# terraytherapeutics/COATI

Measured on AMD Instinct MI355X. Metric: molecules/sec (contrastive+AR train step), grande_closed, higher is better.
Workload: dtype bf16; 1 GPU; grande_closed d=256 L=16 nh=16 + E3GNN h=256x5, V=10322, batch 1024/GPU, seq_len 80, 16-atom point clouds, InfoNCE + AR loss, bf16 MFMA operands / fp32 accumulate + fp32 master weights, random-init weights; global_batch=1024, seq_len=80, parallelism=dp1

## Files before the change

coati_amd/build.py:

```python
import os
import subprocess
import sys
from concurrent.futures import ThreadPoolExecutor

HERE = os.path.dirname(os.path.abspath(__file__))
CSRC = os.path.join(HERE, "csrc")
LIBDIR = os.path.join(HERE, "lib")
LIB = os.path.join(LIBDIR, "libcoati_hip_x.so" if os.environ.get("COATI_AMD_EXPERIMENTAL") == "1" else "libcoati_hip.so")
OBJDIR = os.path.join(HERE, "build")
HIP_UNITS = ["gemm.hip", "gemm_rb.hip", "gemm_rb16.hip", "gemm_ring.hip", "gemm_mx8.hip", "norm.hip", "attention.hip", "attention16.hip", "embed.hip", "gnn.hip", "loss.hip", "optim.hip", "batch.hip", "decode.hip"]
CPP_UNITS = ["engine.cpp", "capi.cpp", "tokenizer.cpp", "comm.cpp"]
FLAGS = ["--offload-arch=gfx950", "-O3", "-std=c++17", "-fPIC", "-Wno-unused-value", "-mllvm", "-amdgpu-mfma-vgpr-form=1"] + os.environ.get("COATI_AMD_CXXFLAGS", "").split()


EXPERIMENTAL = os.environ.get("COATI_AMD_EXPERIMENTAL") == "1"
EXPERIMENTAL_UNITS = ["experimental/attn_block.hip", "experimental/mlp64.hip", "experimental/gemm_t32.hip"]
if EXPERIMENTAL:
    HIP_UNITS = HIP_UNITS + EXPERIMENTAL_UNITS
    FLAGS = FLAGS + ["-DCOATI_EXPERIMENTAL"]
UNIT_DROP_FLAGS = {"experimental/mlp64.hip": ("-mllvm", "-amdgpu-mfma-vgpr-form=1")}


def _hipcc():
    for c in (os.environ.get("HIPCC"), "/opt/rocm/bin/hipcc", "hipcc"):
        if c and (os.path.isabs(c) and os.path.exists(c) or not os.path.isabs(c)):
            return c
    return "hipcc"


def _sources():
    deps = [os.path.join(CSRC, f) for f in os.listdir(CSRC) if not os.path.isdir(os.path.join(CSRC, f))]
    if EXPERIMENTAL:
        deps += [os.path.join(CSRC, "experimental", f) for f in os.listdir(os.path.join(CSRC, "experimental"))]
    deps.append(os.path.join(os.path.dirname(HERE), "include", "coati_hip.h"))
    return deps


def _stamp_path():
    return LIB + ".flags"


def needs_build():
    if not os.path.exists(LIB):
        return True
    try:
        with open(_stamp_path()) as f:
            if f.read() != " ".join(FLAGS):
                return True
    except OSError:
        return True
    t = os.path.getmtime(LIB)
    return any(os.path.getmtime(p) > t for p in _sources())


def build(force=False, verbose=True):
    if not force and not needs_build():
        return LIB
    os.makedirs(LIBDIR, exist_ok=True)
    os.makedirs(OBJDIR, exist_ok=True)
    import fcntl
    with open(os.path.join(LIBDIR, ".build.lock"), "w") as lock:
        fcntl.flock(lock, fcntl.LOCK_EX)
        try:
            if not force and not needs_build():
                return LIB
            return _build_locked(verbose)
        finally:
            fcntl.flock(lock, fcntl.LOCK_UN)


def _build_locked(verbose):
    hipcc = _hipcc()

    def compile_one(unit):
        src = os.path.join(CSRC, unit)
        obj = os.path.join(OBJDIR, unit.replace("/", "_") + (".x.o" if EXPERIMENTAL else ".o"))
        flags = [f for f in FLAGS if f not in UNIT_DROP_FLAGS.get(unit, ())]
        cmd = [hipcc] + flags + (["-x", "hip"] if unit.endswith(".cpp") else []) + ["-c", src, "-o", obj]
        r = subprocess.run(cmd, capture_output=True, text=True)
        if r.returncode != 0:
            raise RuntimeError(f"hipcc failed on {unit}:\n{r.stderr}")
        return obj

    with ThreadPoolExecutor(max_workers=8) as ex:
        objs = list(ex.map(compile_one, HIP_UNITS + CPP_UNITS))
    tmp = LIB + f".tmp{os.getpid()}"
    r = subprocess.run([hipcc, "--offload-arch=gfx950", "-shared", "-fPIC"] + objs + ["-lpthread", "-ldl", "-o", tmp], capture_output=True, text=True)
    if r.returncode != 0:
        raise RuntimeError(f"link failed:\n{r.stderr}")
    os.replace(tmp, LIB)
    with open(_stamp_path(), "w") as f:
        f.write(" ".join(FLAGS))
    if verbose:
        print(f"[coati_amd] built {LIB}", file=sys.stderr)
    return LIB


if __name__ == "__main__":
    build(force="--force" in sys.argv)
```

coati_amd/csrc/engine.cpp:

```cpp
#include <stdarg.h>
#include <stdio.h>
#include <stdlib.h>
#include <string.h>

#include <algorithm>
#include <string>
#include <vector>

#include "../../include/coati_hip.h"
#include "kernels.h"

#define HIPCHK(x) do { hipError_t _h = (x); if (_h != hipSuccess) { coati_set_error("%s: %s", #x, hipGetErrorString(_h)); return COATI_EHIP; } } while (0)

static thread_local char g_err[512] = "";
void coati_set_error(const char* fmt, ...) {
  va_list ap;
  va_start(ap, fmt);
  vsnprintf(g_err, sizeof(g_err), fmt, ap);
  va_end(ap);
}
extern "C" const char* coati_last_error(void) { return g_err; }
extern "C" int coati_abi_version(void) { return COATI_ABI_VERSION; }

namespace {
// ... 229 lines not shown
    x.attnb = c.biases ? add_entry(e, p + "attn.c_attn.bias", 3 * C, 0) : -1;
    x.projw = add_entry(e, p + "attn.c_proj.weight", C, C);
    x.projb = c.biases ? add_entry(e, p + "attn.c_proj.bias", C, 0) : -1;
    x.ln2w = add_entry(e, p + "ln_2.weight", C, 0);
    x.ln2b = add_entry(e, p + "ln_2.bias", C, 0);
    x.fc1w = add_entry(e, p + "mlpf.0.weight", 4 * C, C);
    x.fc1b = c.biases ? add_entry(e, p + "mlpf.0.bias", 4 * C, 0) : -1;
    x.fc2w = add_entry(e, p + "mlpf.2.weight", C, 4 * C);
    x.fc2b = c.biases ? add_entry(e, p + "mlpf.2.bias", C, 0) : -1;
  }
  e->lnfw = add_entry(e, "xformer.transformer.ln_f.weight", C, 0);
  e->lnfb = add_entry(e, "xformer.transformer.ln_f.bias", C, 0);
  if (e->enc_to_coati >= 0) build_layout_coati2_heads(e);
  else build_layout_coati1_heads(e);
  build_layout_shadows(e);
}

void build_layout_coati1_heads(coati_engine* e) {
  const coati_config& c = e->cfg;
  const int C = c.n_hidden_xformer, H = c.n_hidden_e3nn, E = c.n_embd_common, V = c.n_tok;
  auto add_point = [&]() {
    if (c.torch_emb) {
      e->gembw = add_entry(e, "point_encoder.emb.weight", 84, H);
      e->gembb = -1;
    } else {
      e->gembw = add_entry(e, "point_encoder.embedding.weight", H, 28);
      e->gembb = add_entry(e, "point_encoder.embedding.bias", H, 0);
    }
    e->gd0w = add_entry(e, "point_encoder.node_dec.0.weight", H, H);
    e->gd0b = add_entry(e, "point_encoder.node_dec.0.bias", H, 0);
    e->gd3w = add_entry(e, "point_encoder.node_dec.3.weight", H, H);
    e->gd3b = add_entry(e, "point_encoder.node_dec.3.bias", H, 0);
    e->gl.resize(c.n_layer_e3gnn);
    for (int l = 0; l < c.n_layer_e3gnn; ++l) {
      const std::string p = "point_encoder.gcl_" + std::to_string(l) + ".";
      GLayerP& g = e->gl[l];
      g.e0w = add_entry(e, p + "edge_mlp.0.weight", H, 2 * H + 1);
      g.e0b = add_entry(e, p + "edge_mlp.0.bias", H, 0);
      g.e3w = add_entry(e, p + "edge_mlp.3.weight", H, H);
      g.e3b = add_entry(e, p + "edge_mlp.3.bias", H, 0);
      g.n0w = add_entry(e, p + "node_mlp.0.weight", H, 2 * H + (c.residual ? 28 : 0));
      g.n0b = add_entry(e, p + "node_mlp.0.bias", H, 0);
      g.n3w = add_entry(e, p + "node_mlp.3.weight", H, H);
      g.n3b = add_entry(e, p + "node_mlp.3.bias", H, 0);
    }
  };
  auto add_p2c = [&]() {
    if (c.norm_clips && c.old_architecture) {
      e->p2c_w = add_entry(e, "point_to_clip.0.weight", E, H);
      e->p2c_b = add_entry(e, "point_to_clip.0.bias", E, 0);
      e->p2c_lnw = add_entry(e, "point_to_clip.1.weight", H, 0);
      e->p2c_lnb = add_entry(e, "point_to_clip.1.bias", H, 0);
    } else if (c.norm_clips) {
      e->p2c_lnw = add_entry(e, "point_to_clip.0.weight", H, 0);
      e->p2c_lnb = add_entry(e, "point_to_clip.0.bias", H, 0);
      e->p2c_w = add_entry(e, "point_to_clip.1.weight", E, H);
      e->p2c_b = add_entry(e, "point_to_clip.1.bias", E, 0);
    } else {
      e->p2c_w = add_entry(e, "point_to_clip.weight", E, H);
      e->p2c_b = add_entry(e, "point_to_clip.bias", E, 0);
    }
  };
  if (c.use_point_encoder) add_point();
  e->lmhead = add_entry(e, "xformer.lm_head.weight", V, C);
  if (c.use_point_encoder) add_p2c();
  if (c.norm_clips && c.old_architecture) {
    e->s2c_w = add_entry(e, "smiles_to_clip.0.weight", E, C);
    e->s2c_b = add_entry(e, "smiles_to_clip.0.bias", E, 0);
    e->s2c_lnw = add_entry(e, "smiles_to_clip.1.weight", E, 0);
    e->s2c_lnb = add_entry(e, "smiles_to_clip.1.bias", E, 0);
  } else if (c.norm_clips) {
    e->s2c_lnw = add_entry(e, "smiles_to_clip.0.weight", E, 0);
    e->s2c_lnb = add_entry(e, "smiles_to_clip.0.bias", E, 0);
    e->s2c_w = add_entry(e, "smiles_to_clip.1.weight", E, C);
    e->s2c_b = add_entry(e, "smiles_to_clip.1.bias", E, 0);
  } else {
    e->s2c_w = add_entry(e, "smiles_to_clip.weight", E, C);
    e->s2c_b = add_entry(e, "smiles_to_clip.bias", E, 0);
  }
  if (c.token_mlp) {
    e->tokw = add_entry(e, "point_clip_to_special_tokens.1.weight", E, E);
    e->tokb = add_entry(e, "point_clip_to_special_tokens.1.bias", E, 0);
  }
  e->n_trainable = e->n_params;
  if (c.norm_embed) {
    add_entry(e, "xformer.norm_embed.weight", C, 0);
    add_entry(e, "xformer.norm_embed.bias", C, 0);
  }
  if (!c.use_point_encoder) { add_point(); add_p2c(); }
  for (int l = 0; l < c.n_layer_e3gnn; ++l) {
    const std::string p = "point_encoder.gcl_" + std::to_string(l) + ".";
    GLayerP& g = e->gl[l];
    g.c0w = add_entry(e, p + "coord_mlp.0.weight", H, H);
    g.c0b = add_entry(e, p + "coord_mlp.0.bias", H, 0);
    g.c2w = add_entry(e, p + "coord_mlp.2.weight", 1, H);
  }
}

void build_layout_coati2_heads(coati_engine* e) {
  const coati_config& c = e->cfg;
  const int C = c.n_hidden_xformer, E = c.n_embd_common, V = c.n_tok;
  e->lmhead = add_entry(e, "xformer.lm_head.weight", V, C);
  auto swiglu_head = [&](coati_engine::Coati2Head& h, const std::string& p, int i_ln, int i_w1, int i_w2, int d_in, bool residual) {
    h.lnw = add_entry(e, p + std::to_string(i_ln) + ".weight", d_in, 0);
    h.lnb = add_entry(e, p + std::to_string(i_ln) + ".bias", d_in, 0);
    h.w1 = add_entry(e, p + std::to_string(i_w1) + ".weight", 2 * E, d_in);
    h.b1 = add_entry(e, p + std::to_string(i_w1) + ".bias", 2 * E, 0);
    h.w2 = add_entry(e, p + std::to_string(i_w2) + ".weight", E, E);
    h.b2 = add_entry(e, p + std::to_string(i_w2) + ".bias", E, 0);
    h.residual = residual;
  };
  if (e->enc_to_coati == 0) {
    e->s2c_lnw = add_entry(e, "smiles_to_coati.0.weight", E, 0);
    e->s2c_lnb = add_entry(e, "smiles_to_coati.0.bias", E, 0);
    e->s2c_w = add_entry(e, "smiles_to_coati.1.weight", E, C);
    e->s2c_b = add_entry(e, "smiles_to_coati.1.bias", E, 0);
  } else if (e->enc_to_coati == 1) {
    swiglu_head(e->c2s, "smiles_to_coati.", 0, 1, 3, C, false);
  } else {
    swiglu_head(e->c2s, "smiles_to_coati.net.", 0, 2, 4, C, true);
  }
  swiglu_head(e->c2t, "coati_to_token.net.", 0, 2, 4, E, true);
  e->n_trainable = e->n_params;
}

void build_layout_shadows(coati_engine* e) {
  const coati_config& c = e->cfg;
  const int C = c.n_hidden_xformer, H = c.n_hidden_e3nn, V = c.n_tok;
  if (!c.biases) {
    auto hidden = [&](int n) {
      const int64_t off = e->n_params;
      e->n_params = (off + n + 63) & ~(int64_t)63;
      return off;
    };
    for (auto& x : e->xl) { x.attnb = hidden(3 * C); x.projb = hidden(C); x.fc1b = hidden(4 * C); x.fc2b = hidden(C); }
  }

  e->n_shadow = e->n_params;
  for (auto& x : e->xl) {
    x.attnT = add_shadow(e, (int64_t)C * 3 * C);
    x.projT = add_shadow(e, (int64_t)C * C);
    x.fc1T = add_shadow(e, (int64_t)C * 4 * C);
    x.fc2T = add_shadow(e, (int64_t)4 * C * C);
  }
  e->lmheadT = add_shadow(e, (int64_t)C * e->Vpad);
  for (auto& g : e->gl) {
    g.w1ab = add_shadow(e, (int64_t)2 * H * H);
    g.w1abT = add_shadow(e, (int64_t)H * 2 * H);
    g.e3T = add_shadow(e, (int64_t)H * H);
    g.n0T = add_shadow(e, (int64_t)2 * H * H);
    g.n3T = add_shadow(e, (int64_t)H * H);
    g.n0p = c.residual ? add_shadow(e, (int64_t)2 * H * H) : -1;
  }
  if (e->enc_to_coati < 0) {
    e->gd0T = add_shadow(e, (int64_t)H * H);
    e->gd3T = add_shadow(e, (int64_t)H * H);
  }

  e->n_fp8 = 0;
  if (c.use_fp8) {
    for (auto& x : e->xl) {
      const int64_t rows[8] = {3 * C, C, 4 * C, C, C, C, C, 4 * C}, cols[8] = {C, C, C, 4 * C, 3 * C, C, 4 * C, C};
      for (int i = 0; i < 8; ++i) { x.q8[i] = e->n_fp8; e->n_fp8 += (rows[i] * cols[i] + 255) & ~(int64_t)255; }
      for (int i = 0; i < 8; ++i) { x.s8[i] = e->n_fp8; e->n_fp8 += (rows[i] * cols[i] / 32 + 255) & ~(int64_t)255; }
    }
  }

  auto job = [&](int64_t src, int ld_src, int64_t dst, int ld_dst, int rows, int cols, int transpose) {
    e->tile_start.push_back(e->n_job_tiles);
    e->jobs.push_back({src, dst, ld_src, ld_dst, rows, cols, transpose});
    e->n_job_tiles += ((rows + 31) / 32) * ((cols + 31) / 32);
  };
  for (const XLayerP& w : e->xl) {
    job(w.attnw, C, w.attnT, 3 * C, 3 * C, C, 1);
    job(w.projw, C, w.projT, C, C, C, 1);
    job(w.fc1w, C, w.fc1T, 4 * C, 4 * C, C, 1);
    job(w.fc2w, 4 * C, w.fc2T, C, C, 4 * C, 1);
  }
  job(e->lmhead, C, e->lmheadT, e->Vpad, V, C, 1);
  for (const GLayerP& w : e->gl) {
    job(w.e0w, 2 * H + 1, w.w1ab, H, H, H, 0);
    job(w.e0w + H, 2 * H + 1, w.w1ab + (int64_t)H * H, H, H, H, 0);
    job(w.e0w, 2 * H + 1, w.w1abT, 2 * H, H, H, 1);
    job(w.e0w + H, 2 * H + 1, w.w1abT + H, 2 * H, H, H, 1);
    job(w.e3w, H, w.e3T, H, H, H, 1);
    job(w.n0w, 2 * H + (c.residual ? 28 : 0), w.n0T, H, H, 2 * H, 1);
    if (c.residual) job(w.n0w, 2 * H + 28, w.n0p, 2 * H, H, 2 * H, 0);
    job(w.n3w, H, w.n3T, H, H, H, 1);
  }
  if (e->enc_to_coati < 0) {
    job(e->gd0w, H, e->gd0T, H, H, H, 1);
    job(e->gd3w, H, e->gd3T, H, H, H, 1);
  }
}

constexpr int SITE_NONE = -2;
struct ProfScope {
  coati_engine* e;
  hipStream_t s;
  bool on;
  ProfScope(coati_engine* e_, int site, double flops, hipStream_t s_, double bytes = 0.0, double bytes_per_edge = 0.0, double flops_per_edge = 0.0)
      : e(e_), s(s_), on(false) {
    if (site >= 0 && !e->prof_paused && ((e->prof_mask >> site) & 1ull) && e->ev_used + 2 <= (int)e->ev.size()) {
      on = true;
      hipEventRecord(e->ev[e->ev_used], s);
      e->prof_flops += flops;
      e->prof_bytes += bytes;
      e->prof_bytes_e += bytes_per_edge;
      e->prof_flops_e += flops_per_edge;
    }
  }
  ~ProfScope() {
    if (on) {
      hipEventRecord(e->ev[e->ev_used + 1], s);
      e->ev_used += 2;
    }
  }
};

static bool row_split_on() {
  static const bool on = []() { const char* v = getenv("COATI_ROW_SPLIT"); return !(v && v[0] == '0'); }();
  return on;
}
static int row_split_plan(const GemmArgs& a, int a_f32, int epi) {
  if (!row_split_on() || a.m_dev != nullptr || a_f32 || a.M <= 65536 || a.q8_out != nullptr) return 0;
  if (!(a.K == 256 || a.N == 256)) return 0;
  if (epi != EPI_BF16 && epi != EPI_RES_F32 && epi != EPI_QKV_ROPE && epi != EPI_GELU_GRAD && epi != EPI_MUL_AUX && epi != EPI_CE_PARTIAL &&
      epi != EPI_CE_BWD && epi != EPI_CE_BWD_ROW && epi != EPI_LNBWD) return 0;
  long long unit = 16;
  if (epi == EPI_QKV_ROPE && a.rope_row_t == nullptr && a.rope_pos == nullptr && a.rope_T > 0) {
    long long g = unit, t = a.rope_T;
    while (t) { const long long r = g % t; g = t; t = r; }
    unit = unit / g * a.rope_T;
  }
  const int n = cdiv(a.M, 57344);
  const long long rows = (cdiv(a.M, n) + unit - 1) / unit * unit;
  if (rows <= 40960 || rows > 57344 || rows >= a.M) return 0;
  if (epi == EPI_CE_PARTIAL) {
    GemmArgs b = a;
    b.M = (int)rows;
    if (a.partial_tile != 64 || gemm_ce_tile_width(b) != 64) return 0;
  }
  return (int)rows;
}
static void advance_rows(GemmArgs& a, long long r0, int epi, int lnb_partial_rows_done) {
  const bool out32 = (epi == EPI_F32 || epi == EPI_RES_F32 || epi == EPI_ACC_F32 || epi == EPI_LNBWD);
  auto adv = [&](const void* q, long long bytes) -> const void* { return q ? reinterpret_cast<const char*>(q) + bytes : nullptr; };
  a.A = adv(a.A, r0 * a.lda * 2);
  a.C = const_cast<void*>(adv(a.C, r0 * a.ldc * (out32 ? 4 : 2)));
  const long long aux_in_b = (epi == EPI_RES_F32 || epi == EPI_LNBWD) ? 4 : (epi == EPI_MUL_AUX ? 1 : 2);
  const long long aux_out_b = (epi == EPI_GELU_GRAD) ? 1 : 2;
  a.aux_in = adv(a.aux_in, r0 * a.ld_aux * aux_in_b);
  a.aux_out = const_cast<void*>(adv(a.aux_out, r0 * a.ld_aux * aux_out_b));
  if (a.lse) a.lse += r0;
  if (a.target) a.target += r0;
  if (a.row_scale) a.row_scale += r0;
  if (a.partial) a.partial += r0 * cdiv(a.N, a.partial_tile > 0 ? a.partial_tile : 128);
  if (a.rope_row_t) a.rope_row_t += r0;
  if (a.ln_x) { a.ln_x += r0 * a.ln_ldx; a.ln_mean += r0; a.ln_rstd += r0; }
  if (a.lnb_x) { a.lnb_x += r0 * a.lnb_ldx; a.lnb_mean += r0; a.lnb_rstd += r0; }
  if (a.lnb_partial) a.lnb_partial += (long long)lnb_partial_rows_done * 2 * a.N;
  if (a.chain_C) a.chain_C += r0 * a.chain_ldc;
}
static int gemm_rows(const GemmArgs& a, int a_f32, int epi, hipStream_t s, int* lnb_rows = nullptr) {
  const int rows = row_split_plan(a, a_f32, epi);
  if (rows == 0) {
    if (lnb_rows) { int nwg = 0; gemm_ring_lnbwd_supported(a, &nwg); *lnb_rows = nwg; }
    return launch_gemm_nt(a, a_f32, epi, s);
  }
  int done = 0;
  for (long long r0 = 0; r0 < a.M; r0 += rows) {
    GemmArgs b = a;
    b.M = (int)std::min<long long>(rows, a.M - r0);
    advance_rows(b, r0, epi, done);
    if (epi == EPI_LNBWD) {
      int nwg = 0;
      if (!gemm_ring_lnbwd_supported(b, &nwg)) { coati_set_error("gemm_rows: a row range of %d rows does not take the fused LayerNorm backward", b.M); return COATI_ESHAPE; }
      done += nwg;
    }
    COATI_TRY(launch_gemm_nt(b, a_f32, epi, s));
  }
  if (lnb_rows) *lnb_rows = done;
  return COATI_OK;
}
static bool lnbwd_rows_supported(const GemmArgs& a, int* nwg) {
  const int rows = row_split_plan(a, 0, EPI_LNBWD);
  if (rows == 0) return gemm_ring_lnbwd_supported(a, nwg);
  int total = 0;
  for (long long r0 = 0; r0 < a.M; r0 += rows) {
    GemmArgs b = a;
    b.M = (int)std::min<long long>(rows, a.M - r0);
    int k = 0;
    if (!gemm_ring_lnbwd_supported(b, &k)) return false;
    total += k;
  }
  if (nwg) *nwg = total;
  return true;
}

static bool gnn_edge_fused_on() {
  static const bool on = []() { const char* v = getenv("COATI_GNN_EDGE_FUSED"); return !(v && v[0] == '0'); }();
  return on;
}
static bool lpt_on() {
  static const bool on = []() { const char* v = getenv("COATI_ATTN_LPT"); return !(v && v[0] == '0'); }();
  return on;
}
int gemm(coati_engine* e, int site, const void* A, int a_f32, int64_t lda, const bf16_t* Bm, int64_t ldb, int M,
         int N, int K, void* Cm, int64_t ldc, const float* bias, int epi, const void* aux_in, void* aux_out,
         int64_t ld_aux, hipStream_t s) {
  GemmArgs a;
  memset(&a, 0, sizeof(a));
  a.A = A; a.lda = lda; a.B = Bm; a.ldb = ldb; a.M = M; a.N = N; a.K = K; a.C = Cm; a.ldc = ldc; a.bias = bias;
  a.aux_in = aux_in; a.aux_out = aux_out; a.ld_aux = ld_aux;
  const bool out32 = (epi == EPI_F32 || epi == EPI_RES_F32 || epi == EPI_ACC_F32);
  double bytes = (double)M * K * (a_f32 ? 4 : 2) + (double)N * K * 2 + (double)M * N * (out32 ? 4 : 2);
  if (epi == EPI_RES_F32 || epi == EPI_ACC_F32) bytes += (double)M * N * 4;
  if (epi == EPI_GELU || epi == EPI_SILU || epi == EPI_DGELU || epi == EPI_DSILU) bytes += (double)M * N * 2;
  if (epi == EPI_GELU_GRAD || epi == EPI_MUL_AUX) bytes += (double)M * N;
  ProfScope ps(e, site, 2.0 * M * N * K, s, bytes);
  return gemm_rows(a, a_f32, epi, s);
}
int wgrad(coati_engine* e, int site, const void* A, int a_f32, int64_t lda, const bf16_t* Bm, int64_t ldb, int M,
          int N, int K, float* dW, int64_t ldw, float* dbias, int n_out, hipStream_t s) {
  WgradArgs a;
  a.A = A; a.lda = lda; a.B = Bm; a.ldb = ldb; a.M = M; a.N = N; a.K = K; a.dW = dW; a.ldw = ldw; a.dbias = dbias;
  a.n_out = n_out;
  ProfScope ps(e, site, 2.0 * M * N * K, s, (double)M * N * (a_f32 ? 4 : 2) + (double)M * K * 2 + (double)N * K * 8);
  return launch_wgrad(a, a_f32, s);
}

int gemm8(coati_engine* e, int site, const XLayerP& w, int wi, const bf16_t* A, int64_t lda, int M, int N, int K, GemmArgs a, int epi, hipStream_t s,
          bool emit = false) {
  COATI_CHECK_ARG(e->S8 && e->q8, "fp8 mode: coati_engine_bind_fp8 has not been called");
  const bool pre = A == nullptr;
  a.A = pre ? e->q8b : e->q8; a.lda = K; a.B = reinterpret_cast<const bf16_t*>(e->S8 + w.q8[wi]); a.ldb = K; a.M = M; a.N = N; a.K = K;
  if (emit) { a.q8_out = e->q8b; a.q8_scales = e->q8bs; a.ld_q8 = N; }
  const bool out32 = (epi == EPI_F32 || epi == EPI_RES_F32);
  double bytes = (pre ? 0.0 : (double)M * K * 3) + (double)M * K * (1.0 + 1.0 / 32) + (double)N * K * (1.0 + 1.0 / 32) + (double)M * N * (out32 ? 4 : 2);
  if (epi == EPI_RES_F32) bytes += (double)M * N * 4;
  if (epi == EPI_GELU_GRAD || epi == EPI_MUL_AUX) bytes += (double)M * N;
  if (emit) bytes += (double)M * N * (1.0 + 1.0 / 32);
  ProfScope ps(e, site, 2.0 * M * N * K, s, bytes);
  if (!pre) COATI_TRY(launch_quant_mx8(A, 0, lda, e->q8, K, e->q8s, M, K, s));
  return launch_gemm_mx8(a, pre ? e->q8bs : e->q8s, e->S8 + w.s8[wi], epi, s);
}

void carve_pass(coati_engine* e, Arena& ar, XPass& p, int B_, int T_, int B, int T) {
  const int L = e->cfg.n_layer_xformer, C = e->cfg.n_hidden_xformer, nh = e->cfg.n_head;
  const size_t M = (size_t)B * T;
  p.B = B_; p.T = T_; p.M = B_ * T_; p.Mcap = (int)M;
  p.x.assign(L + 1, nullptr); p.xmid.assign(L, nullptr);
  p.mean1.assign(L, nullptr); p.rstd1.assign(L, nullptr); p.mean2.assign(L, nullptr); p.rstd2.assign(L, nullptr);
  p.lse.assign(L, nullptr);
  p.a1.assign(L, nullptr); p.qkv.assign(L, nullptr); p.y.assign(L, nullptr); p.a2.assign(L, nullptr);
  p.hpre.assign(L, nullptr); p.g.assign(L, nullptr);
  for (int l = 0; l <= L; ++l) p.x[l] = ar.take<float>(M * C);
  for (int l = 0; l < L; ++l) {
    p.xmid[l] = ar.take<float>(M * C);
    p.mean1[l] = ar.take<float>(M); p.rstd1[l] = ar.take<float>(M);
    p.mean2[l] = ar.take<float>(M); p.rstd2[l] = ar.take<float>(M);
    p.lse[l] = ar.take<float>((size_t)B * nh * T);
    p.a1[l] = ar.take<bf16_t>(M * C);
    p.qkv[l] = ar.take<bf16_t>(M * 3 * C);
    p.y[l] = ar.take<bf16_t>(M * C);
    p.a2[l] = ar.take<bf16_t>(M * C);
    p.hpre[l] = ar.take<unsigned char>(M * 4 * C);
    p.g[l] = ar.take<bf16_t>(M * 4 * C);
  }
  p.meanf = ar.take<float>(M); p.rstdf = ar.take<float>(M);
  p.xf32 = ar.take<float>(M * C);
  if (e->cfg.norm_embed) { p.x_emb = ar.take<float>(M * C); p.mean0 = ar.take<float>(M); p.rstd0 = ar.take<float>(M); }
  p.af = ar.take<bf16_t>(M * C);
  p.t_xmid = ar.take<float>((size_t)B * C); p.t_xL = ar.take<float>((size_t)B * C); p.t_xf = ar.take<float>((size_t)B * C);
  p.t_mean2 = ar.take<float>(B); p.t_rstd2 = ar.take<float>(B); p.t_meanf = ar.take<float>(B); p.t_rstdf = ar.take<float>(B);
  p.t_a2 = ar.take<bf16_t>((size_t)B * C); p.t_g = ar.take<bf16_t>((size_t)B * 4 * C); p.t_hpre = ar.take<unsigned char>((size_t)B * 4 * C);
  p.tail = false;
  p.packed = false;
  p.off = ar.take<int>((size_t)B + 1); p.ord = ar.take<int>((size_t)B); p.row_src = ar.take<int>(M); p.row_t = ar.take<int>(M); p.ypk = ar.take<long long>(M);
  p.grp = ar.take<int>((size_t)B + 2);
}

size_t carve(coati_engine* e, Arena& ar, int B_, int T1_, int T2_, int A_, int Bg) {
  const coati_config& c = e->cfg;
  const int B = B_ > e->cap_B ? B_ : e->cap_B, T1 = T1_ > e->cap_T1 ? T1_ : e->cap_T1, T2 = T2_ > e->cap_T2 ? T2_ : e->cap_T2,
            A = A_ > e->cap_A ? A_ : e->cap_A;
  const int C = c.n_hidden_xformer, H = c.n_hidden_e3nn, E = c.n_embd_common, Lg = c.n_layer_e3gnn;
  const size_t Mmax = (size_t)B * (T1 > T2 ? T1 : T2), M2 = (size_t)B * T2;
  const size_t BA = (size_t)B * A, Me = BA * A;
  carve_pass(e, ar, e->p1, B_, T1_, B, T1);
  carve_pass(e, ar, e->p2, B_, T2_, B, T2);
  e->hpoint = ar.take<float>((size_t)B * H); e->hp_ln = ar.take<float>((size_t)B * H);
  e->hp_mean = ar.take<float>(B); e->hp_rstd = ar.take<float>(B);
  e->hstop = ar.take<float>((size_t)B * C); e->hs_ln = ar.take<float>((size_t)B * C);
  e->hs_mean = ar.take<float>(B); e->hs_rstd = ar.take<float>(B);
  e->h_e3gnn = ar.take<float>((size_t)B * E); e->h_smiles = ar.take<float>((size_t)B * E);
  e->sa = ar.take<float>((size_t)B * E); e->sb = ar.take<float>((size_t)B * E);
  e->ptok = ar.take<float>((size_t)B * E); e->stok = ar.take<float>((size_t)B * E);
  e->cliptok = ar.take<float>((size_t)B * E);
  e->ones = ar.take<float>(B);
  e->stop_pos = ar.take<int>(B);
  e->err_flag = ar.take<int>(4);
  if (e->enc_to_coati >= 0) e->c2_u = ar.take<float>((size_t)B * 2 * E);
  const int tiles_v = cdiv(c.n_tok, 64);
  e->ce_partial = ar.take<float2>(M2 * tiles_v);
  e->ce_lse = ar.take<float>(M2);
  e->dlogits = ar.take<bf16_t>(M2 * e->Vpad);
  e->g_h32.assign(Lg + 1, nullptr); e->g_rstd.assign(Lg + 1, nullptr);
  e->g_hcat.assign(Lg, nullptr); e->g_P.assign(Lg, nullptr); e->g_e1.assign(Lg, nullptr); e->g_s2.assign(Lg, nullptr);
  e->g_upre.assign(Lg, nullptr); e->g_t.assign(Lg, nullptr);
  for (int l = 0; l <= Lg; ++l) { e->g_h32[l] = ar.take<float>(BA * H); e->g_rstd[l] = ar.take<float>(BA); }
  for (int l = 0; l < Lg; ++l) {
    e->g_hcat[l] = ar.take<bf16_t>(BA * 2 * H); e->g_P[l] = ar.take<bf16_t>(BA * 2 * H);
    e->g_e1[l] = ar.take<bf16_t>(Me * H); e->g_s2[l] = ar.take<bf16_t>(Me * H);
    e->g_upre[l] = ar.take<bf16_t>(BA * H); e->g_t[l] = ar.take<bf16_t>(BA * H);
  }
  e->g_hfin16 = ar.take<bf16_t>(BA * H); e->g_dpre = ar.take<bf16_t>(BA * H); e->g_td = ar.take<bf16_t>(BA * H);
  e->g_mask = ar.take<float>(BA); e->g_d2 = ar.take<float>(Me); e->g_w = ar.take<float>(Me);
  e->g_seg = ar.take<int>(BA + 1); e->g_ne = ar.take<int>(4); e->g_ebj = ar.take<int>(Me); e->g_ebk = ar.take<int>(Me);
  e->g_erev = ar.take<int>(Me); e->g_pos = ar.take<int>(Me); e->g_ed2 = ar.take<float>(Me); e->g_ew = ar.take<float>(Me);
  e->g_o = ar.take<float>(BA * H); e->g_o2 = ar.take<float>(BA * H);
  e->DX = ar.take<float>(Mmax * C);
  e->DX16 = ar.take<bf16_t>(Mmax * C);
  e->g_DO16 = ar.take<bf16_t>(BA * H);
  e->dh4 = ar.take<bf16_t>(Mmax * 4 * C); e->da = ar.take<bf16_t>(Mmax * C); e->dyb = ar.take<bf16_t>(Mmax * C);
  e->dqkv = ar.take<bf16_t>(Mmax * 3 * C);
  e->attnD = ar.take<float>(Mmax * c.n_head);
  e->dcliptok = ar.take<float>((size_t)B * E); e->dptok = ar.take<float>((size_t)B * E); e->dstok = ar.take<float>((size_t)B * E);
  e->dsa = ar.take<float>((size_t)B * E); e->dsb = ar.take<float>((size_t)B * E);
  e->dhe = ar.take<float>((size_t)B * E); e->dhs = ar.take<float>((size_t)B * E);
  e->dhs_ln = ar.take<float>((size_t)B * C); e->dhstop = ar.take<float>((size_t)B * C);
  e->dhp_ln = ar.take<float>((size_t)B * H); e->dhpoint = ar.take<float>((size_t)B * H);
  e->g_DH = ar.take<float>(BA * H); e->g_DO = ar.take<float>(BA * H);
  e->g_do2 = ar.take<bf16_t>(BA * H); e->g_dtd = ar.take<bf16_t>(BA * H); e->g_du = ar.take<bf16_t>(BA * H);
  e->g_dmi = ar.take<bf16_t>(BA * H); e->g_ds2 = ar.take<bf16_t>(Me * H); e->g_dpre1 = ar.take<bf16_t>(Me * H);
  e->g_dP = ar.take<bf16_t>(BA * 2 * H);
  e->t_dx = ar.take<float>((size_t)B * C); e->t_dxa = ar.take<bf16_t>((size_t)B * C); e->t_dxb = ar.take<bf16_t>((size_t)B * C);
  e->t_dh4 = ar.take<bf16_t>((size_t)B * 4 * C); e->t_da = ar.take<bf16_t>((size_t)B * C);
  {
    const int L = c.n_layer_xformer;
    e->wg_group = C % 128 == 0 && Mmax >= 4096;
    e->wg_tile = (C % 256 == 0 && 40LL * 4 * C < (1LL << 30)) ? 256 : 128;
    e->w_dh4.assign(L, nullptr); e->w_dxa.assign(L, nullptr); e->w_dxb.assign(L, nullptr); e->w_dqkv.assign(L, nullptr);
    if (e->wg_group) {
      for (int l = 0; l < L; ++l) {
        e->w_dh4[l] = ar.take<bf16_t>(Mmax * 4 * C); e->w_dxa[l] = ar.take<bf16_t>(Mmax * C);
        e->w_dxb[l] = ar.take<bf16_t>(Mmax * C); e->w_dqkv[l] = ar.take<bf16_t>(Mmax * 3 * C);
      }
      const int tpl = cdiv(3 * C, 128) * cdiv(C, 128) + cdiv(C, 128) * cdiv(C, 128) + 2 * cdiv(4 * C, 128) * cdiv(C, 128);
      e->wtab_cap = L * tpl;
      WgradTile* t = ar.take<WgradTile>((size_t)4 * e->wtab_cap);
      if (t != e->d_wtab || ar.base != e->wtab_ws) for (auto& k : e->wtab_key) k = coati_engine::WTabKey();
      e->d_wtab = t;
      e->wtab_ws = ar.base;
    }
    const long long csig = (((long long)B * 1000003 + T1) * 1000003 + T2) * 1000003 + A;
    if (!e->wg_group || csig != e->carve_sig) for (auto& k : e->wtab_key) k = coati_engine::WTabKey();
    {
      e->gnn_wg_group = H % 128 == 0 && BA >= 4096 && Lg > 0;
      e->gl_DO16.assign(Lg, nullptr); e->gl_du.assign(Lg, nullptr); e->gl_dP.assign(Lg, nullptr);
      if (e->gnn_wg_group) {
        for (int l = 0; l < Lg; ++l) { e->gl_DO16[l] = ar.take<bf16_t>(BA * H); e->gl_du[l] = ar.take<bf16_t>(BA * H); e->gl_dP[l] = ar.take<bf16_t>(BA * 2 * H); }
        e->gtab_cap = 4 * (2 + Lg * 5) * cdiv(H, 128) * cdiv(H, 128);
        WgradTile* t = ar.take<WgradTile>((size_t)e->gtab_cap);
        if (t != e->d_gtab || ar.base != e->gtab_ws || csig != e->carve_sig) e->gtab_sig = -1;
        e->d_gtab = t;
        e->gtab_ws = ar.base;
      } else {
        e->gtab_sig = -1;
      }
    }
    e->carve_sig = csig;
  }
  if (c.use_fp8) {
    e->q8 = ar.take<unsigned char>(Mmax * 4 * C);
    e->q8s = ar.take<unsigned char>(Mmax * 4 * C / 32);
    e->q8b = ar.take<unsigned char>(Mmax * 4 * C);
    e->q8bs = ar.take<unsigned char>(Mmax * 4 * C / 32);
  }
  e->ce_rowscale = ar.take<float>(M2);
  e->opt_partial = ar.take<float>(1024);
  e->ln_partial = ar.take<float>((size_t)COATI_LN_PARTIAL_ROWS * 2 * (C > H ? C : H));
  e->ln_part_x = ar.take<float>((size_t)(2 * c.n_layer_xformer + 1) * COATI_LN_PARTIAL_ROWS * 2 * C);
  {
    ShadowJob* dj = ar.take<ShadowJob>(e->jobs.size());
    int* dt = ar.take<int>(e->tile_start.size());
    if (dj != e->d_jobs || dt != e->d_tile_start) e->jobs_uploaded = false;
    e->d_jobs = dj; e->d_tile_start = dt;
  }
  e->nce_cap = (size_t)2 * B_ * (Bg > B_ ? Bg : B_);
  e->nce = ar.take<float>(e->nce_cap);
  return (ar.off + 255) & ~(size_t)255;
}

int xformer_fwd(coati_engine* e, XPass& p, const float* injection, hipStream_t s) {
  const coati_config& c = e->cfg;
  const int C = c.n_hidden_xformer, L = c.n_layer_xformer, M = p.M;
  {
    ProfScope ps(e, SITE_EMBED, 0, s);
    if (c.norm_embed) {
      COATI_TRY(launch_embed_fwd(p.idx, e->P + e->tok_emb, nullptr, c.unk_token, p.x_emb, p.B, p.T, C, c.n_tok, s, p.packed ? p.row_src : nullptr, M));
      COATI_TRY(launch_layernorm_fwd(p.x_emb, C, e->P + e->emb_lnw, e->P + e->emb_lnb, nullptr, 0, p.x[0], C, p.mean0, p.rstd0, M, C, s));
      if (injection != nullptr)
        COATI_TRY(launch_embed_fwd(p.idx, nullptr, injection, c.unk_token, p.x[0], p.B, p.T, C, c.n_tok, s, p.packed ? p.row_src : nullptr, M, 1));
    } else {
      COATI_TRY(launch_embed_fwd(p.idx, e->P + e->tok_emb, injection, c.unk_token, p.x[0], p.B, p.T, C, c.n_tok, s, p.packed ? p.row_src : nullptr, M));
    }
  }
#ifdef COATI_EXPERIMENTAL
  const bool ab = !c.use_fp8 && attn_block_fwd_supported(p.B, p.T, C, c.n_head);
  if (ab) COATI_TRY(launch_attn_groups(p.packed ? p.off : nullptr, p.B, p.T, p.grp, s));
#else
  constexpr bool ab = false;
#endif
  for (int l = 0; l < L; ++l) {
    const XLayerP& w = e->xl[l];
#ifdef COATI_EXPERIMENTAL
    if (ab) {
      AttnBlockArgs a;
      a.x = p.x[l]; a.xmid = p.xmid[l]; a.ln_g = e->P + w.ln1w; a.ln_b = e->P + w.ln1b; a.mean = p.mean1[l]; a.rstd = p.rstd1[l];
      a.a1 = p.a1[l]; a.Wqkv = e->S + w.attnw; a.bqkv = e->P + w.attnb; a.Wproj = e->S + w.projw; a.bproj = e->P + w.projb;
      a.qkv = p.qkv[l]; a.y = p.y[l]; a.lse = p.lse[l]; a.cos_t = e->cos_t; a.sin_t = e->sin_t; a.row_src = p.packed ? p.row_src : nullptr;
      a.grp = p.grp; a.Tl = p.T; a.M = M;
      ProfScope ps(e, SITE_ATTN_BLOCK_FWD, 2.0 * M * 4 * C * C + 4.0 * M * (double)p.T * C, s,
                   (double)M * C * (4 + 2 + 6 + 2 + 4) + (double)M * (c.n_head * 4 + 8) + 4.0 * C * C * 2);
      COATI_TRY(launch_attn_block_fwd(a, s));
    }
#endif
    if (c.use_fp8) {
      GemmArgs a;
      {
        ProfScope ps(e, SITE_LN_FWD, 0, s, (double)M * C * 6 + (double)M * 8);
        COATI_TRY(launch_layernorm_fwd(p.x[l], C, e->P + w.ln1w, e->P + w.ln1b, p.a1[l], C, nullptr, 0, p.mean1[l], p.rstd1[l], M, C, s));
      }
      memset(&a, 0, sizeof(a));
      a.C = p.qkv[l]; a.ldc = 3 * C; a.bias = e->P + w.attnb; a.rope_cos = e->cos_t; a.rope_sin = e->sin_t; a.rope_T = p.T; a.rope_C = C;
      a.rope_hs = C / c.n_head; a.rope_row_t = p.packed ? p.row_t : nullptr;
      COATI_TRY(gemm8(e, SITE_QKV_FWD, w, 0, p.a1[l], C, M, 3 * C, C, a, EPI_QKV_ROPE, s));
      {
        ProfScope ps(e, SITE_ATTN_FWD, 4.0 * M * (double)p.T * C, s, (double)M * 4 * C * 2 + (double)M * c.n_head * 4);
        COATI_TRY(launch_attn_fwd(p.qkv[l], p.y[l], p.lse[l], p.B, p.T, c.n_head, C / c.n_head, s, p.packed ? p.off : nullptr, p.packed && lpt_on() ? p.ord : nullptr));
      }
      memset(&a, 0, sizeof(a));
      a.C = p.xmid[l]; a.ldc = C; a.bias = e->P + w.projb; a.aux_in = p.x[l]; a.ld_aux = C;
      COATI_TRY(gemm8(e, SITE_PROJ_FWD, w, 1, p.y[l], C, M, C, C, a, EPI_RES_F32, s));
      {
        ProfScope ps(e, SITE_LN_FWD, 0, s, (double)M * C * 6 + (double)M * 8);
        COATI_TRY(launch_layernorm_fwd(p.xmid[l], C, e->P + w.ln2w, e->P + w.ln2b, p.a2[l], C, nullptr, 0, p.mean2[l], p.rstd2[l], M, C, s));
      }
      memset(&a, 0, sizeof(a));
      a.C = p.g[l]; a.ldc = 4 * C; a.bias = e->P + w.fc1b; a.aux_out = p.hpre[l]; a.ld_aux = 4 * C;
      COATI_TRY(gemm8(e, SITE_FC1_FWD, w, 2, p.a2[l], C, M, 4 * C, C, a, EPI_GELU_GRAD, s, true));
      memset(&a, 0, sizeof(a));
      a.C = p.x[l + 1]; a.ldc = C; a.bias = e->P + w.fc2b; a.aux_in = p.xmid[l]; a.ld_aux = C;
      COATI_TRY(gemm8(e, SITE_FC2_FWD, w, 3, nullptr, 4 * C, M, C, 4 * C, a, EPI_RES_F32, s));
      continue;
    }
    if (!ab) {
      GemmArgs a;
      memset(&a, 0, sizeof(a));
      a.A = p.a1[l]; a.lda = C; a.B = e->S + w.attnw; a.ldb = C; a.M = M; a.N = 3 * C; a.K = C; a.C = p.qkv[l]; a.ldc = 3 * C;
      a.bias = e->P + w.attnb; a.rope_cos = e->cos_t; a.rope_sin = e->sin_t; a.rope_T = p.T; a.rope_C = C; a.rope_hs = C / c.n_head;
      a.rope_row_t = p.packed ? p.row_t : nullptr;
      const bool fuse = gemm_rb256_ln_fusable(a, EPI_QKV_ROPE);
      if (fuse) {
        a.ln_x = p.x[l]; a.ln_ldx = C; a.ln_gamma = e->P + w.ln1w; a.ln_beta = e->P + w.ln1b; a.ln_mean = p.mean1[l]; a.ln_rstd = p.rstd1[l];
      } else {
        ProfScope ps(e, SITE_LN_FWD, 0, s, (double)M * C * 6 + (double)M * 8);
        COATI_TRY(launch_layernorm_fwd(p.x[l], C, e->P + w.ln1w, e->P + w.ln1b, p.a1[l], C, nullptr, 0, p.mean1[l], p.rstd1[l], M, C, s));
      }
      ProfScope ps(e, SITE_QKV_FWD, 2.0 * M * 3 * C * C, s, (double)M * C * (fuse ? 6 : 2) + 3.0 * C * C * 2 + (double)M * 3 * C * 2);
      COATI_TRY(gemm_rows(a, 0, EPI_QKV_ROPE, s));
    }
    if (!ab) {
      {
        ProfScope ps(e, SITE_ATTN_FWD, 4.0 * M * (double)p.T * C, s, (double)M * 4 * C * 2 + (double)M * c.n_head * 4);
        COATI_TRY(launch_attn_fwd(p.qkv[l], p.y[l], p.lse[l], p.B, p.T, c.n_head, C / c.n_head, s, p.packed ? p.off : nullptr, p.packed && lpt_on() ? p.ord : nullptr));
      }
      COATI_TRY(gemm(e, SITE_PROJ_FWD, p.y[l], 0, C, e->S + w.projw, C, M, C, C, p.xmid[l], C, e->P + w.projb, EPI_RES_F32, p.x[l], nullptr, C, s));
    }
    if (p.tail && l == L - 1) {
      const int B = p.B;
      COATI_TRY(launch_gather_rows(p.xmid[l], e->stop_pos, p.t_xmid, B, p.T, C, s, p.packed ? p.off : nullptr));
      {
        ProfScope ps(e, SITE_XF_TAIL, 0, s, (double)B * C * 6 + (double)B * 8);
        COATI_TRY(launch_layernorm_fwd(p.t_xmid, C, e->P + w.ln2w, e->P + w.ln2b, p.t_a2, C, nullptr, 0, p.t_mean2, p.t_rstd2, B, C, s));
      }
      COATI_TRY(gemm(e, SITE_XF_TAIL, p.t_a2, 0, C, e->S + w.fc1w, C, B, 4 * C, C, p.t_g, 4 * C, e->P + w.fc1b, EPI_GELU_GRAD, nullptr, p.t_hpre, 4 * C, s));
      COATI_TRY(gemm(e, SITE_XF_TAIL, p.t_g, 0, 4 * C, e->S + w.fc2w, 4 * C, B, C, 4 * C, p.t_xL, C, e->P + w.fc2b, EPI_RES_F32, p.t_xmid, nullptr, C, s));
      ProfScope ps(e, SITE_XF_TAIL, 0, s, (double)B * C * 8 + (double)B * 8);
      return launch_layernorm_fwd(p.t_xL, C, e->P + e->lnfw, e->P + e->lnfb, nullptr, 0, p.t_xf, C, p.t_meanf, p.t_rstdf, B, C, s);
    }
    {
      GemmArgs a;
      memset(&a, 0, sizeof(a));
      a.A = p.a2[l]; a.lda = C; a.B = e->S + w.fc1w; a.ldb = C; a.M = M; a.N = 4 * C; a.K = C; a.C = p.g[l]; a.ldc = 4 * C;
      a.bias = e->P + w.fc1b; a.aux_out = p.hpre[l]; a.ld_aux = 4 * C;
      const bool fuse = gemm_rb256_ln_fusable(a, EPI_GELU_GRAD);
      if (fuse) {
        a.ln_x = p.xmid[l]; a.ln_ldx = C; a.ln_gamma = e->P + w.ln2w; a.ln_beta = e->P + w.ln2b; a.ln_mean = p.mean2[l]; a.ln_rstd = p.rstd2[l];
      } else {
        ProfScope ps(e, SITE_LN_FWD, 0, s, (double)M * C * 6 + (double)M * 8);
        COATI_TRY(launch_layernorm_fwd(p.xmid[l], C, e->P + w.ln2w, e->P + w.ln2b, p.a2[l], C, nullptr, 0, p.mean2[l], p.rstd2[l], M, C, s));
      }
      ProfScope ps(e, SITE_FC1_FWD, 2.0 * M * 4 * C * C, s, (double)M * C * (fuse ? 6 : 2) + 4.0 * C * C * 2 + (double)M * 4 * C * 3);
      COATI_TRY(gemm_rows(a, 0, EPI_GELU_GRAD, s));
    }
    COATI_TRY(gemm(e, SITE_FC2_FWD, p.g[l], 0, 4 * C, e->S + w.fc2w, 4 * C, M, C, 4 * C, p.x[l + 1], C, e->P + w.fc2b, EPI_RES_F32, p.xmid[l], nullptr, C, s));
  }
  float* const y32 = (&p == &e->p1) ? p.xf32 : nullptr;
  ProfScope ps(e, SITE_LN_FWD, 0, s, (double)M * C * (y32 ? 8 : 6) + (double)M * 8);
  return launch_layernorm_fwd(p.x[L], C, e->P + e->lnfw, e->P + e->lnfb, y32 ? nullptr : p.af, C, y32, C, p.meanf, p.rstdf, M, C, s);
}

int upload_table(coati_engine* e, int hslot, const std::vector<WgradTile>& tab, WgradTile* dst, hipStream_t s, const char* what) {
  const size_t n = tab.size();
  if (e->h_tab_ev[hslot] == nullptr && hipEventCreateWithFlags(&e->h_tab_ev[hslot], hipEventDisableTiming) != hipSuccess) {
    coati_set_error("%s: event creation failed", what);
    return COATI_EHIP;
  } else if (e->h_tab[hslot] != nullptr && hipEventSynchronize(e->h_tab_ev[hslot]) != hipSuccess) {
    coati_set_error("%s: waiting for the previous upload failed", what);
    return COATI_EHIP;
  }
  if (e->h_tab_cap[hslot] < n) {
    if (e->h_tab[hslot] != nullptr) hipHostFree(e->h_tab[hslot]);
    e->h_tab[hslot] = nullptr;
    if (hipHostMalloc(reinterpret_cast<void**>(&e->h_tab[hslot]), n * sizeof(WgradTile), hipHostMallocDefault) != hipSuccess) {
      coati_set_error("%s: pinned staging allocation failed", what);
      return COATI_EHIP;
    }
    e->h_tab_cap[hslot] = n;
  }
  memcpy(e->h_tab[hslot], tab.data(), n * sizeof(WgradTile));
  if (hipMemcpyAsync(dst, e->h_tab[hslot], n * sizeof(WgradTile), hipMemcpyHostToDevice, s) != hipSuccess || hipEventRecord(e->h_tab_ev[hslot], s) != hipSuccess) {
    coati_set_error("%s: table upload failed", what);
    return COATI_EHIP;
  }
  return COATI_OK;
}

int xformer_wgrad_group(coati_engine* e, XPass& p, int l_lo, int l_hi, hipStream_t s) {
  const int C = e->cfg.n_hidden_xformer, M = p.M, Mtab = p.Mcap;
  const long long sig = e->carve_sig * 2 + (p.tail ? 1 : 0);
  int slot = -1;
  for (int i = 0; i < 4; ++i)
    if (e->wtab_key[i].pass == &p && e->wtab_key[i].lo == l_lo && e->wtab_key[i].hi == l_hi && e->wtab_key[i].M == Mtab && e->wtab_key[i].sig == sig) slot = i;
  double flops = 0.0, bytes = 0.0;
  for (int l = l_lo; l < l_hi; ++l) {
    flops += 2.0 * M * (3.0 + 1.0 + 4.0 + 4.0) * C * C;
    bytes += (double)M * (3 + 1 + 1 + 1 + 4 + 1 + 1 + 4) * C * 2 + 12.0 * C * C * 8;
  }
  if (slot < 0) {
    std::vector<WgradTile> tab;
    auto add = [&](const bf16_t* A, int lda, const bf16_t* B, int ldb, int N, int K, int64_t w_off, int64_t b_off) -> int {
      WgradArgs a;
      a.A = A; a.lda = lda; a.B = B; a.ldb = ldb; a.M = Mtab; a.N = N; a.K = K; a.dW = e->G + w_off; a.ldw = K; a.dbias = e->G + b_off; a.n_out = 0;
      return wgrad_table_append(tab, a, e->wg_tile);
    };
    for (int l = l_hi - 1; l >= l_lo; --l) {
      const XLayerP& w = e->xl[l];
      COATI_TRY(add(e->w_dqkv[l], 3 * C, p.a1[l], C, 3 * C, C, w.attnw, w.attnb));
      COATI_TRY(add(e->w_dxb[l], C, p.y[l], C, C, C, w.projw, w.projb));
      if (p.tail && l == e->cfg.n_layer_xformer - 1) continue;
      COATI_TRY(add(e->w_dh4[l], 4 * C, p.a2[l], C, 4 * C, C, w.fc1w, w.fc1b));
      COATI_TRY(add(e->w_dxa[l], C, p.g[l], 4 * C, C, 4 * C, w.fc2w, w.fc2b));
    }
    COATI_CHECK_ARG((int)tab.size() <= e->wtab_cap, "wgrad group: table overflow (%zu > %d)", tab.size(), e->wtab_cap);
    slot = e->wtab_rr++ & 3;
    COATI_TRY(upload_table(e, slot, tab, e->d_wtab + (size_t)slot * e->wtab_cap, s, "wgrad group"));
    coati_engine::WTabKey k;
    k.pass = &p; k.lo = l_lo; k.hi = l_hi; k.M = Mtab; k.n = (int)tab.size(); k.sig = sig;
    e->wtab_key[slot] = k;
  }
  ProfScope ps(e, SITE_XF_WGRAD, flops, s, bytes);
  return launch_wgrad_table(e->d_wtab + (size_t)slot * e->wtab_cap, e->wtab_key[slot].n, s, e->wg_tile, M);
}

int xformer_bwd(coati_engine* e, XPass& p, const void* dyf, int dyf_f32, float* dinjection, hipStream_t s, int l_hi = -1, int l_lo = 0,
                const bf16_t* lmh_dlogits = nullptr, bool inputs_only = false) {
  const coati_config& c = e->cfg;
  const int C = c.n_hidden_xformer, L = c.n_layer_xformer, M = p.M;
  if (l_hi < 0) l_hi = L;
  float* DX = e->DX;
  const bool defer = 2 * L + 1 <= COATI_LN_MAX_SLOTS;
  const long long slot_stride = (long long)COATI_LN_PARTIAL_ROWS * 2 * C;
  LnFinishBatch fin;
  memset(&fin, 0, sizeof(fin));
  int nblk = 0;
  auto ln_bwd = [&](const void* dy, int dy_f32, const float* x, const float* mean, const float* rstd, const float* gamma,
                    const float* dres, size_t goff, size_t boff, bf16_t* dx16) -> int {
    if (!defer && inputs_only) return launch_layernorm_bwd(dy, dy_f32, C, x, C, 0, mean, rstd, gamma, dres, DX, dx16, nullptr, nullptr, e->ln_partial, M, C, s);
    if (!defer) return launch_layernorm_bwd(dy, dy_f32, C, x, C, 0, mean, rstd, gamma, dres, DX, dx16, e->G + goff, e->G + boff, e->ln_partial, M, C, s);
    fin.dg_off[fin.n] = (long long)goff;
    fin.db_off[fin.n] = (long long)boff;
    return launch_layernorm_bwd_deferred(dy, dy_f32, C, x, C, 0, mean, rstd, gamma, dres, DX, dx16, e->ln_part_x + (fin.n++) * slot_stride, &nblk, M, C, s);
  };
  auto dgrad_lnbwd = [&](int site, const bf16_t* dY, int K, const bf16_t* WT, const float* x, const float* mean, const float* rstd,
                         const float* gamma, size_t goff, size_t boff, bf16_t* dx16, const bf16_t* chainW = nullptr,
                         bf16_t* chainC = nullptr, bool has_dres = true) -> int {
    if (!defer || c.use_fp8) return 0;
    GemmArgs a;
    memset(&a, 0, sizeof(a));
    a.A = dY; a.lda = K; a.B = WT; a.ldb = K; a.M = M; a.N = C; a.K = K; a.C = DX; a.ldc = C; a.aux_in = has_dres ? DX : nullptr; a.ld_aux = C; a.aux_out = dx16;
    a.lnb_x = x; a.lnb_ldx = C; a.lnb_mean = mean; a.lnb_rstd = rstd; a.lnb_gamma = gamma;
    if (chainW != nullptr && dx16 != nullptr) { a.chain_W = chainW; a.chain_ldw = C; a.chain_C = chainC; a.chain_ldc = C; }
    int nwg = 0;
    if (!lnbwd_rows_supported(a, &nwg) || nwg > COATI_LN_PARTIAL_ROWS) return 0;
    a.lnb_partial = e->ln_part_x + fin.n * slot_stride;
    fin.dg_off[fin.n] = (long long)goff;
    fin.db_off[fin.n] = (long long)boff;
    fin.nblk[fin.n] = nwg;
    ++fin.n;
    ProfScope ps(e, site, 2.0 * M * C * K + (a.chain_W ? 2.0 * M * C * C : 0.0), s,
                 (double)M * K * 2 + (double)C * K * 2 + (double)M * C * (4 + (has_dres ? 4 : 0) + 4 + (dx16 ? 2 : 0)) + (a.chain_W ? (double)M * C * 2 + (double)C * C * 2 : 0.0));
    const int rc = gemm_rows(a, 0, EPI_LNBWD, s);
    return rc == COATI_OK ? 1 : rc;
  };
  const bool grp = e->wg_group && M >= 4096 && !inputs_only;
  const bool wg_each = !grp && !inputs_only;
  COATI_CHECK_ARG(!inputs_only || (!p.tail && !c.use_fp8 && dinjection != nullptr), "xformer_bwd: the inputs-only backward serves a full bf16 pass with an injection");
  if (l_hi == L && p.tail) {
    ProfScope ps(e, SITE_XF_TAIL, 0, s, (double)p.B * C * ((dyf_f32 ? 4 : 2) + 4 + 4 + 2));
    COATI_TRY(launch_layernorm_bwd(dyf, dyf_f32, C, p.t_xL, C, 0, p.t_meanf, p.t_rstdf, e->P + e->lnfw, nullptr, e->t_dx, e->t_dxa, e->G + e->lnfw, e->G + e->lnfb, e->ln_partial, p.B, C, s));
  } else if (l_hi == L) {
    int lnf_fused = 0;
    if (lmh_dlogits != nullptr) {
      lnf_fused = dgrad_lnbwd(SITE_LMHEAD_DGRAD, lmh_dlogits, e->Vpad, e->S + e->lmheadT, p.x[L], p.meanf, p.rstdf, e->P + e->lnfw, e->lnfw, e->lnfb,
                              grp ? e->w_dxa[L - 1] : e->DX16, nullptr, nullptr, false);
      if (lnf_fused < 0) return lnf_fused;
      if (!lnf_fused) COATI_TRY(gemm(e, SITE_LMHEAD_DGRAD, lmh_dlogits, 0, e->Vpad, e->S + e->lmheadT, e->Vpad, M, C, e->Vpad, e->da, C, nullptr, EPI_BF16, nullptr, nullptr, 0, s));
    }
    if (!lnf_fused) {
      ProfScope ps(e, SITE_LN_BWD, 0, s, (double)M * C * ((dyf_f32 ? 4 : 2) + 4 + 4 + 2));
      COATI_TRY(ln_bwd(dyf, dyf_f32, p.x[L], p.meanf, p.rstdf, e->P + e->lnfw, nullptr, e->lnfw, e->lnfb, grp ? e->w_dxa[L - 1] : e->DX16));
    }
  }
  for (int l = l_hi - 1; l >= l_lo; --l) {
    const XLayerP& w = e->xl[l];
    bf16_t* const dxa = grp ? e->w_dxa[l] : e->DX16;
    bf16_t* const dxb = grp ? e->w_dxb[l] : e->DX16;
    bf16_t* const dh4 = grp ? e->w_dh4[l] : e->dh4;
    bf16_t* const dqkv = grp ? e->w_dqkv[l] : e->dqkv;
    bf16_t* const dx_out = l == 0 ? nullptr : (grp ? e->w_dxa[l - 1] : e->DX16);
    int ln2_fused = 0, ln1_fused = 0;
    if (p.tail && l == L - 1) {
      const int Bt = p.B;
      COATI_TRY(gemm(e, SITE_XF_TAIL, e->t_dxa, 0, C, e->S + w.fc2T, C, Bt, 4 * C, C, e->t_dh4, 4 * C, nullptr, EPI_MUL_AUX, p.t_hpre, nullptr, 4 * C, s));
      COATI_TRY(gemm(e, SITE_XF_TAIL, e->t_dh4, 0, 4 * C, e->S + w.fc1T, 4 * C, Bt, C, 4 * C, e->t_da, C, nullptr, EPI_BF16, nullptr, nullptr, 0, s));
      COATI_TRY(wgrad(e, SITE_XF_TAIL, e->t_dh4, 0, 4 * C, p.t_a2, C, Bt, 4 * C, C, e->G + w.fc1w, C, e->G + w.fc1b, 0, s));
      COATI_TRY(wgrad(e, SITE_XF_TAIL, e->t_dxa, 0, C, p.t_g, 4 * C, Bt, C, 4 * C, e->G + w.fc2w, 4 * C, e->G + w.fc2b, 0, s));
      {
        ProfScope ps(e, SITE_XF_TAIL, 0, s, (double)Bt * C * (2 + 4 + 4 + 4 + 2));
        COATI_TRY(launch_layernorm_bwd(e->t_da, 0, C, p.t_xmid, C, 0, p.t_mean2, p.t_rstd2, e->P + w.ln2w, e->t_dx, e->t_dx, e->t_dxb, e->G + w.ln2w, e->G + w.ln2b, e->ln_partial, Bt, C, s));
        if (hipMemsetAsync(DX, 0, (size_t)M * C * sizeof(float), s) != hipSuccess || hipMemsetAsync(dxb, 0, (size_t)M * C * sizeof(bf16_t), s) != hipSuccess) {
          coati_set_error("xformer_bwd: hipMemsetAsync failed");
          return COATI_EHIP;
        }
        COATI_TRY(launch_scatter_rows_add(e->t_dx, e->stop_pos, DX, Bt, p.T, C, s, p.packed ? p.off : nullptr));
        COATI_TRY(launch_scatter_rows_bf16(e->t_dxb, e->stop_pos, dxb, Bt, p.T, C, s, p.packed ? p.off : nullptr));
      }
    } else {
      if (c.use_fp8) {
        GemmArgs a;
        memset(&a, 0, sizeof(a));
        a.C = dh4; a.ldc = 4 * C; a.aux_in = p.hpre[l]; a.ld_aux = 4 * C;
        COATI_TRY(gemm8(e, SITE_FC2_DGRAD, w, 7, dxa, C, M, 4 * C, C, a, EPI_MUL_AUX, s, true));
        memset(&a, 0, sizeof(a));
        a.C = e->da; a.ldc = C;
        COATI_TRY(gemm8(e, SITE_FC1_DGRAD, w, 6, nullptr, 4 * C, M, C, 4 * C, a, EPI_BF16, s));
      } else {
      COATI_TRY(gemm(e, SITE_FC2_DGRAD, dxa, 0, C, e->S + w.fc2T, C, M, 4 * C, C, dh4, 4 * C, nullptr, EPI_MUL_AUX, p.hpre[l], nullptr, 4 * C, s));
      ln2_fused = dgrad_lnbwd(SITE_FC1_DGRAD, dh4, 4 * C, e->S + w.fc1T, p.xmid[l], p.mean2[l], p.rstd2[l], e->P + w.ln2w, w.ln2w, w.ln2b, dxb,
                              e->S + w.projT, e->dyb);
      if (ln2_fused < 0) return ln2_fused;
      if (!ln2_fused) COATI_TRY(gemm(e, SITE_FC1_DGRAD, dh4, 0, 4 * C, e->S + w.fc1T, 4 * C, M, C, 4 * C, e->da, C, nullptr, EPI_BF16, nullptr, nullptr, 0, s));
      }
      if (wg_each) {
        COATI_TRY(wgrad(e, SITE_XF_WGRAD, dh4, 0, 4 * C, p.a2[l], C, M, 4 * C, C, e->G + w.fc1w, C, e->G + w.fc1b, 0, s));
        COATI_TRY(wgrad(e, SITE_XF_WGRAD, dxa, 0, C, p.g[l], 4 * C, M, C, 4 * C, e->G + w.fc2w, 4 * C, e->G + w.fc2b, 0, s));
      }
      if (!ln2_fused) {
        ProfScope ps(e, SITE_LN_BWD, 0, s, (double)M * C * (2 + 4 + 4 + 4 + 2));
        COATI_TRY(ln_bwd(e->da, 0, p.xmid[l], p.mean2[l], p.rstd2[l], e->P + w.ln2w, DX, w.ln2w, w.ln2b, dxb));
      }
    }
    if (c.use_fp8) {
      GemmArgs a;
      memset(&a, 0, sizeof(a));
      a.C = e->dyb; a.ldc = C;
      COATI_TRY(gemm8(e, SITE_PROJ_DGRAD, w, 5, dxb, C, M, C, C, a, EPI_BF16, s));
    } else if (!ln2_fused) {
    COATI_TRY(gemm(e, SITE_PROJ_DGRAD, dxb, 0, C, e->S + w.projT, C, M, C, C, e->dyb, C, nullptr, EPI_BF16, nullptr, nullptr, 0, s));
    }
    if (wg_each) COATI_TRY(wgrad(e, SITE_XF_WGRAD, dxb, 0, C, p.y[l], C, M, C, C, e->G + w.projw, C, e->G + w.projb, 0, s));
    {
      ProfScope ps(e, SITE_ATTN_BWD, 10.0 * M * (double)p.T * C, s, (double)M * 8 * C * 2 + (double)M * c.n_head * 8);
      COATI_TRY(launch_attn_bwd(p.qkv[l], p.y[l], e->dyb, p.lse[l], e->attnD, dqkv, e->cos_t, e->sin_t, p.B, p.T, c.n_head, C / c.n_head, s, p.packed ? p.off : nullptr, p.packed && lpt_on() ? p.ord : nullptr));
    }
    if (c.use_fp8) {
      GemmArgs a;
      memset(&a, 0, sizeof(a));
      a.C = e->da; a.ldc = C;
      COATI_TRY(gemm8(e, SITE_QKV_DGRAD, w, 4, dqkv, 3 * C, M, C, 3 * C, a, EPI_BF16, s));
    } else {
    ln1_fused = dgrad_lnbwd(SITE_QKV_DGRAD, dqkv, 3 * C, e->S + w.attnT, p.x[l], p.mean1[l], p.rstd1[l], e->P + w.ln1w, w.ln1w, w.ln1b, dx_out);
    if (ln1_fused < 0) return ln1_fused;
    if (!ln1_fused) COATI_TRY(gemm(e, SITE_QKV_DGRAD, dqkv, 0, 3 * C, e->S + w.attnT, 3 * C, M, C, 3 * C, e->da, C, nullptr, EPI_BF16, nullptr, nullptr, 0, s));
    }
    if (wg_each) COATI_TRY(wgrad(e, SITE_XF_WGRAD, dqkv, 0, 3 * C, p.a1[l], C, M, 3 * C, C, e->G + w.attnw, C, e->G + w.attnb, 0, s));
    if (!ln1_fused) {
      ProfScope ps(e, SITE_LN_BWD, 0, s, (double)M * C * (2 + 4 + 4 + 4 + 2));
      COATI_TRY(ln_bwd(e->da, 0, p.x[l], p.mean1[l], p.rstd1[l], e->P + w.ln1w, DX, w.ln1w, w.ln1b, dx_out));
    }
  }
  if (grp && l_hi > l_lo) COATI_TRY(xformer_wgrad_group(e, p, l_lo, l_hi, s));
  if (defer && fin.n > 0 && !inputs_only) {
    ProfScope ps(e, SITE_LN_BWD, 0, s, 0.0);
    COATI_TRY(launch_ln_finish_batched(e->ln_part_x, slot_stride, nblk, e->G, fin, C, s));
  }
  if (l_lo > 0) return COATI_OK;
  ProfScope ps(e, SITE_EMBED, 0, s);
  if (inputs_only) return launch_embed_bwd(p.idx, DX, nullptr, dinjection, c.unk_token, p.B, p.T, C, c.n_tok, s, p.packed ? p.off : nullptr, 1);
  if (c.norm_embed) {
    if (dinjection != nullptr) {
      COATI_TRY(launch_embed_bwd(p.idx, DX, nullptr, dinjection, c.unk_token, p.B, p.T, C, c.n_tok, s, p.packed ? p.off : nullptr, 1));
      COATI_TRY(launch_embed_fwd(p.idx, nullptr, nullptr, c.unk_token, DX, p.B, p.T, C, c.n_tok, s, p.packed ? p.row_src : nullptr, M, 2));
    }
    COATI_TRY(launch_layernorm_bwd(DX, 1, C, p.x_emb, C, 0, p.mean0, p.rstd0, e->P + e->emb_lnw, nullptr, p.x[0], nullptr, e->G + e->emb_lnw, e->G + e->emb_lnb,
                                   e->ln_partial, M, C, s));
    return launch_embed_bwd(p.idx, p.x[0], e->G + e->tok_emb, nullptr, c.unk_token, p.B, p.T, C, c.n_tok, s, p.packed ? p.off : nullptr);
  }
  return launch_embed_bwd(p.idx, DX, e->G + e->tok_emb, dinjection, c.unk_token, p.B, p.T, C, c.n_tok, s, p.packed ? p.off : nullptr);
}

int gnn_fwd(coati_engine* e, const long long* atoms, const float* coords, hipStream_t s) {
  const coati_config& c = e->cfg;
  const int H = c.n_hidden_e3nn, Lg = c.n_layer_e3gnn, B = e->B, A = e->A, BA = B * A, Me = BA * A;
  {
    ProfScope ps(e, SITE_GNN_ELEMWISE, 0, s, (double)BA * (8 + H * 6 + 8) + (double)BA * 12 + (double)Me * 8 * 3 + (double)BA * 4, 20.0);
    bf16_t* h16 = Lg > 0 ? e->g_hcat[0] : e->g_hfin16;
    if (c.torch_emb) COATI_TRY(launch_gnn_embed(atoms, nullptr, nullptr, e->P + e->gembw, nullptr, e->g_h32[0], h16, Lg > 0 ? 2 * H : H, e->g_rstd[0], e->g_mask, BA, H, s, e->err_flag));
    else COATI_TRY(launch_gnn_embed(atoms, e->lut_ix, e->lut_iy, e->P + e->gembw, e->P + e->gembb, e->g_h32[0], h16, Lg > 0 ? 2 * H : H, e->g_rstd[0], e->g_mask, BA, H, s));
    COATI_TRY(launch_gnn_geom(coords, e->g_mask, c.msg_cutoff, e->g_d2, e->g_w, B, A, s));
    COATI_TRY(launch_gnn_compact(e->g_w, e->g_d2, e->g_seg, e->g_ne, e->g_ebj, e->g_ebk, e->g_erev, e->g_ed2, e->g_ew, e->g_pos, B, A, s));
  }
  for (int l = 0; l < Lg; ++l) {
    const GLayerP& w = e->gl[l];
    COATI_TRY(gemm(e, SITE_GNN_NODE_GEMM, e->g_hcat[l], 0, 2 * H, e->S + w.w1ab, H, BA, 2 * H, H, e->g_P[l], 2 * H, nullptr, EPI_BF16, nullptr, nullptr, 0, s));
    if (H == 256 && gnn_edge_fused_on()) {
      ProfScope ps(e, SITE_GNN_EDGE_GEMM, 0, s, (double)BA * (H * 2 + 4 + H * 2) + (double)H * H * 2, (double)H * 2 + 12 + (double)H * 4, 2.0 * H * H + 6.0 * H);
      COATI_TRY(launch_gnn_edge_fwd_fused(e->g_P[l], 2 * H, e->g_seg, e->g_ebk, e->g_ed2, e->g_ew, e->P + w.e0w + 2 * H, 2 * H + 1, e->P + w.e0b,
                                          e->S + w.e3w, H, e->P + w.e3b, e->g_e1[l], e->g_s2[l], e->g_hcat[l] + H, 2 * H, BA, H, s));
    } else {
    {
      ProfScope ps(e, SITE_GNN_ELEMWISE, 0, s, (double)BA * (H * 2 + 4), (double)H * 4 + 8, 4.0 * H);
      COATI_TRY(launch_gnn_edge_pre_c(e->g_P[l], 2 * H, e->g_seg, e->g_ebk, e->g_ed2, e->P + w.e0w + 2 * H, 2 * H + 1, e->P + w.e0b, e->g_e1[l], BA, H, s));
    }
    {
      GemmArgs a;
      memset(&a, 0, sizeof(a));
      a.m_dev = e->g_ne;
      a.A = e->g_e1[l]; a.lda = H; a.B = e->S + w.e3w; a.ldb = H; a.M = Me; a.N = H; a.K = H; a.C = e->g_s2[l]; a.ldc = H; a.bias = e->P + w.e3b;
      ProfScope ps(e, SITE_GNN_EDGE_GEMM, 0, s, (double)H * H * 2 + H * 4, (double)H * 4, 2.0 * H * H);
      COATI_TRY(launch_gemm_nt(a, 0, EPI_BF16, s));
    }
    {
      ProfScope ps(e, SITE_GNN_ELEMWISE, 0, s, (double)BA * (H * 2 + 4), (double)H * 2 + 4, 2.0 * H);
      COATI_TRY(launch_gnn_edge_reduce_c(e->g_s2[l], e->g_seg, e->g_ew, e->g_hcat[l] + H, 2 * H, BA, H, s));
    }
    }
    if (c.residual) {
      COATI_TRY(gemm(e, SITE_GNN_NODE_GEMM, e->g_hcat[l], 0, 2 * H, e->S + w.n0p, 2 * H, BA, H, 2 * H, e->g_o, H, e->P + w.n0b, EPI_F32, nullptr, nullptr, 0, s));
      ProfScope ps(e, SITE_GNN_ELEMWISE, 0, s, (double)BA * (H * 4 + 8 + H * 4));
      COATI_TRY(launch_gnn_node_res_silu(e->g_o, atoms, e->lut_ix, e->lut_iy, e->P + w.n0w + 2 * H, 2 * H + 28, e->g_upre[l], e->g_t[l], BA, H, s));
    } else {
      COATI_TRY(gemm(e, SITE_GNN_NODE_GEMM, e->g_hcat[l], 0, 2 * H, e->S + w.n0w, 2 * H, BA, H, 2 * H, e->g_t[l], H, e->P + w.n0b, EPI_SILU, nullptr, e->g_upre[l], H, s));
    }
    COATI_TRY(gemm(e, SITE_GNN_NODE_GEMM, e->g_t[l], 0, H, e->S + w.n3w, H, BA, H, H, e->g_o, H, e->P + w.n3b, EPI_RES_F32, e->g_h32[l], nullptr, H, s));
    {
      ProfScope ps(e, SITE_GNN_ELEMWISE, 0, s, (double)BA * (H * 4 + H * 4 + H * 2 + 4));
      const bool last = (l + 1 == Lg);
      COATI_TRY(launch_layernorm_fwd(e->g_o, H, nullptr, nullptr, last ? e->g_hfin16 : e->g_hcat[l + 1], last ? H : 2 * H, e->g_h32[l + 1], H, nullptr, e->g_rstd[l + 1], BA, H, s));
    }
  }
  COATI_TRY(gemm(e, SITE_GNN_NODE_GEMM, e->g_hfin16, 0, H, e->S + e->gd0w, H, BA, H, H, e->g_td, H, e->P + e->gd0b, EPI_SILU, nullptr, e->g_dpre, H, s));
  COATI_TRY(gemm(e, SITE_GNN_NODE_GEMM, e->g_td, 0, H, e->S + e->gd3w, H, BA, H, H, e->g_o2, H, e->P + e->gd3b, EPI_F32, nullptr, nullptr, 0, s));
  ProfScope ps(e, SITE_GNN_ELEMWISE, 0, s, (double)BA * (H * 4 + 4) + (double)B * H * 4);
  return launch_gnn_readout(e->g_o2, e->g_mask, e->hpoint, B, A, H, s);
}

int gnn_wgrad_group(coati_engine* e, hipStream_t s) {
  const coati_config& c = e->cfg;
  const int H = c.n_hidden_e3nn, Lg = c.n_layer_e3gnn, BA = e->B * e->A;
  const long long sig = (e->carve_sig * 1000003 + e->B) * 1000003 + e->A;
  if (e->gtab_sig != sig) {
    std::vector<WgradTile> tab;
    auto add = [&](const bf16_t* A_, int lda, const bf16_t* B_, int ldb, int N, int K, float* dW, int64_t ldw, float* db) -> int {
      WgradArgs a;
      a.A = A_; a.lda = lda; a.B = B_; a.ldb = ldb; a.M = BA; a.N = N; a.K = K; a.dW = dW; a.ldw = ldw; a.dbias = db; a.n_out = 0;
      return wgrad_table_append_split(tab, a, 4);
    };
    COATI_TRY(add(e->g_do2, H, e->g_td, H, H, H, e->G + e->gd3w, H, e->G + e->gd3b));
    COATI_TRY(add(e->g_dtd, H, e->g_hfin16, H, H, H, e->G + e->gd0w, H, e->G + e->gd0b));
    for (int l = Lg - 1; l >= 0; --l) {
      const GLayerP& w = e->gl[l];
      COATI_TRY(add(e->gl_DO16[l], H, e->g_t[l], H, H, H, e->G + w.n3w, H, e->G + w.n3b));
      COATI_TRY(add(e->gl_du[l], H, e->g_hcat[l], 2 * H, H, 2 * H, e->G + w.n0w, 2 * H + (c.residual ? 28 : 0), e->G + w.n0b));
      COATI_TRY(add(e->gl_dP[l], 2 * H, e->g_hcat[l], 2 * H, H, H, e->G + w.e0w, 2 * H + 1, nullptr));
      COATI_TRY(add(e->gl_dP[l] + H, 2 * H, e->g_hcat[l], 2 * H, H, H, e->G + w.e0w + H, 2 * H + 1, nullptr));
    }
    COATI_CHECK_ARG((int)tab.size() <= e->gtab_cap, "gnn wgrad group: table overflow (%zu > %d)", tab.size(), e->gtab_cap);
    COATI_TRY(upload_table(e, 4 + (e->gtab_rr++ & 1), tab, e->d_gtab, s, "gnn wgrad group"));
    e->gtab_n = (int)tab.size();
    e->gtab_sig = sig;
  }
  const double nprob = 2.0 + 4.0 * Lg + Lg;
  ProfScope ps(e, SITE_GNN_WGRAD, 2.0 * BA * H * H * nprob, s, nprob * ((double)BA * H * 4 + (double)H * H * 8));
  return launch_wgrad_split_table(e->d_gtab, e->gtab_n, s);
}

int gnn_bwd(coati_engine* e, const float* dhpoint, hipStream_t s) {
  const coati_config& c = e->cfg;
  const int H = c.n_hidden_e3nn, Lg = c.n_layer_e3gnn, B = e->B, A = e->A, BA = B * A, Me = BA * A;
  float *DH = e->g_DH, *DO = e->g_DO;
  const bool grp = e->gnn_wg_group;
  {
    ProfScope ps(e, SITE_GNN_ELEMWISE, 0, s, (double)B * H * 4 + (double)BA * (H * 2 + 4));
    COATI_TRY(launch_gnn_readout_bwd(dhpoint, e->g_mask, e->g_do2, B, A, H, s));
  }
  COATI_TRY(gemm(e, SITE_GNN_NODE_GEMM, e->g_do2, 0, H, e->S + e->gd3T, H, BA, H, H, e->g_dtd, H, nullptr, EPI_DSILU, e->g_dpre, nullptr, H, s));
  if (!grp) COATI_TRY(wgrad(e, SITE_GNN_WGRAD, e->g_do2, 0, H, e->g_td, H, BA, H, H, e->G + e->gd3w, H, e->G + e->gd3b, 0, s));
  COATI_TRY(gemm(e, SITE_GNN_NODE_GEMM, e->g_dtd, 0, H, e->S + e->gd0T, H, BA, H, H, DH, H, nullptr, EPI_F32, nullptr, nullptr, 0, s));
  if (!grp) COATI_TRY(wgrad(e, SITE_GNN_WGRAD, e->g_dtd, 0, H, e->g_hfin16, H, BA, H, H, e->G + e->gd0w, H, e->G + e->gd0b, 0, s));
  for (int l = Lg - 1; l >= 0; --l) {
    const GLayerP& w = e->gl[l];
    bf16_t* const DO16 = grp ? e->gl_DO16[l] : e->g_DO16;
    bf16_t* const du = grp ? e->gl_du[l] : e->g_du;
    bf16_t* const dP = grp ? e->gl_dP[l] : e->g_dP;
    {
      ProfScope ps(e, SITE_GNN_ELEMWISE, 0, s, (double)BA * (H * 4 + H * 4 + 4 + H * 4 + H * 2));
      COATI_TRY(launch_layernorm_bwd(DH, 1, H, e->g_h32[l + 1], H, 1, nullptr, e->g_rstd[l + 1], nullptr, nullptr, DO, DO16, nullptr, nullptr, e->ln_partial, BA, H, s));
    }
    COATI_TRY(gemm(e, SITE_GNN_NODE_GEMM, DO16, 0, H, e->S + w.n3T, H, BA, H, H, du, H, nullptr, EPI_DSILU, e->g_upre[l], nullptr, H, s));
    if (!grp) COATI_TRY(wgrad(e, SITE_GNN_WGRAD, DO16, 0, H, e->g_t[l], H, BA, H, H, e->G + w.n3w, H, e->G + w.n3b, 0, s));
    COATI_TRY(gemm(e, SITE_GNN_NODE_GEMM, du, 0, H, e->S + w.n0T, H, BA, H, H, DO, H, nullptr, EPI_ACC_F32, nullptr, nullptr, 0, s));
    COATI_TRY(gemm(e, SITE_GNN_NODE_GEMM, du, 0, H, e->S + w.n0T + (int64_t)H * H, H, BA, H, H, e->g_dmi, H, nullptr, EPI_BF16, nullptr, nullptr, 0, s));
    if (!grp) COATI_TRY(wgrad(e, SITE_GNN_WGRAD, du, 0, H, e->g_hcat[l], 2 * H, BA, H, 2 * H, e->G + w.n0w, 2 * H + (c.residual ? 28 : 0), e->G + w.n0b, 0, s));
    if (c.residual) {
      ProfScope ps(e, SITE_GNN_ELEMWISE, 0, s, (double)BA * (H * 2 + 8));
      COATI_TRY(launch_gnn_onehot_wgrad(e->atoms, e->lut_ix, e->lut_iy, du, e->G + w.n0w + 2 * H, 2 * H + 28, BA, H, s));
    }
    {
      ProfScope ps(e, SITE_GNN_ELEMWISE, 0, s, (double)BA * (H * 2 + 4), (double)H * 4 + 4, 6.0 * H);
      COATI_TRY(launch_gnn_edge_reduce_bwd_c(e->g_dmi, H, e->g_s2[l], e->g_seg, e->g_ew, e->g_ds2, BA, H, s));
    }
    {
      GemmArgs a;
      memset(&a, 0, sizeof(a));
      a.A = e->g_ds2; a.lda = H; a.B = e->S + w.e3T; a.ldb = H; a.M = Me; a.N = H; a.K = H; a.C = e->g_dpre1; a.ldc = H;
      a.P = e->g_P[l]; a.ldp = 2 * H; a.d2 = e->g_ed2; a.w1c = e->P + w.e0w + 2 * H; a.w1c_stride = 2 * H + 1;
      a.b1 = e->P + w.e0b; a.natom = A; a.H = H;
      a.m_dev = e->g_ne; a.e_bj = e->g_ebj; a.e_bk = e->g_ebk;
      ProfScope ps(e, SITE_GNN_EDGE_GEMM, 0, s, (double)H * H * 2, (double)H * 8 + 12, 2.0 * H * H + 8.0 * H);
      COATI_TRY(launch_gemm_nt(a, 0, EPI_EDGE_DPRE, s));
    }
    {
      WgradArgs a;
      a.A = e->g_ds2; a.lda = H; a.B = e->g_e1[l]; a.ldb = H; a.M = Me; a.N = H; a.K = H; a.dW = e->G + w.e3w; a.ldw = H; a.dbias = e->G + w.e3b;
      a.n_out = 0; a.m_dev = e->g_ne;
      ProfScope ps(e, SITE_GNN_WGRAD, 0, s, (double)H * H * 8, (double)H * 4, 2.0 * H * H);
      COATI_TRY(launch_wgrad(a, 0, s));
    }
    {
      ProfScope ps(e, SITE_GNN_ELEMWISE, 0, s, (double)BA * (H * 4 + 4), (double)H * 4 + 8, 4.0 * H);
      COATI_TRY(launch_gnn_edge_pre_bwd_c(e->g_dpre1, e->g_seg, e->g_erev, e->g_ed2, dP, 2 * H, e->G + w.e0w + 2 * H, 2 * H + 1, e->G + w.e0b, BA, H, s));
    }
    COATI_TRY(gemm(e, SITE_GNN_NODE_GEMM, dP, 0, 2 * H, e->S + w.w1abT, 2 * H, BA, H, 2 * H, DO, H, nullptr, EPI_ACC_F32, nullptr, nullptr, 0, s));
    if (!grp) {
      COATI_TRY(wgrad(e, SITE_GNN_WGRAD, dP, 0, 2 * H, e->g_hcat[l], 2 * H, BA, H, H, e->G + w.e0w, 2 * H + 1, nullptr, 0, s));
      COATI_TRY(wgrad(e, SITE_GNN_WGRAD, dP + H, 0, 2 * H, e->g_hcat[l], 2 * H, BA, H, H, e->G + w.e0w + H, 2 * H + 1, nullptr, 0, s));
    }
    float* t = DH; DH = DO; DO = t;
  }
  if (grp) COATI_TRY(gnn_wgrad_group(e, s));
  {
    ProfScope ps(e, SITE_GNN_ELEMWISE, 0, s, (double)BA * (H * 4 + H * 4 + 4 + H * 4) + (double)BA * (8 + H * 4) + 30.0 * H * 4);
    COATI_TRY(launch_layernorm_bwd(DH, 1, H, e->g_h32[0], H, 1, nullptr, e->g_rstd[0], nullptr, nullptr, DO, nullptr, nullptr, nullptr, e->ln_partial, BA, H, s));
    if (e->cfg.torch_emb) COATI_TRY(launch_gnn_embed_bwd(e->atoms, nullptr, nullptr, DO, e->G + e->gembw, nullptr, BA, H, s));
    else COATI_TRY(launch_gnn_embed_bwd(e->atoms, e->lut_ix, e->lut_iy, DO, e->G + e->gembw, e->G + e->gembb, BA, H, s));
  }
  return COATI_OK;
}

int head_linear_bwd(coati_engine* e, SgemmBatch& sb, const float* dY, const float* X, int64_t w_off, int64_t b_off, float* dX, int B,
                    int N, int K) {
  const float* W = e->P + w_off;
  COATI_TRY(sgemm_batch_add(sb, dY, 1, N, X, K, 1, e->G + w_off, K, N, K, B, nullptr, 1.f, 1));
  COATI_TRY(sgemm_batch_add(sb, e->ones, 0, 1, dY, N, 1, e->G + b_off, N, 1, N, B, nullptr, 1.f, 1));
  if (dX) COATI_TRY(sgemm_batch_add(sb, dY, N, 1, W, K, 1, dX, K, B, K, N, nullptr, 1.f, 0));
  return COATI_OK;
}

int ensure_side(coati_engine* e) {
  if (e->side) return COATI_OK;
  if (hipStreamCreateWithFlags(&e->side, hipStreamNonBlocking) != hipSuccess ||
      hipEventCreateWithFlags(&e->ev_fork, hipEventDisableTiming) != hipSuccess ||
      hipEventCreateWithFlags(&e->ev_join, hipEventDisableTiming) != hipSuccess) {
    coati_set_error("engine: could not create the side stream");
    return COATI_EHIP;
  }
  return COATI_OK;
}
int fork_side(coati_engine* e, hipStream_t main) {
  COATI_TRY(ensure_side(e));
  if (hipEventRecord(e->ev_fork, main) != hipSuccess || hipStreamWaitEvent(e->side, e->ev_fork, 0) != hipSuccess) {
    coati_set_error("engine: fork failed");
    return COATI_EHIP;
  }
  return COATI_OK;
}
int join_side(coati_engine* e, hipStream_t main) {
  if (hipEventRecord(e->ev_join, e->side) != hipSuccess || hipStreamWaitEvent(main, e->ev_join, 0) != hipSuccess) {
    coati_set_error("engine: join failed");
    return COATI_EHIP;
  }
  return COATI_OK;
}

int point_head_fwd(coati_engine* e, float* out, hipStream_t s) {
  const coati_config& c = e->cfg;
  const int H = c.n_hidden_e3nn, E = c.n_embd_common, B = e->B;
  if (!c.use_point_encoder) return COATI_OK;
  const float* x = e->hpoint;
  if (c.norm_clips && c.old_architecture) {
    COATI_TRY(launch_sgemm(x, H, 1, e->P + e->p2c_w, 1, H, e->hp_ln, E, B, E, H, e->P + e->p2c_b, 1.f, 0, s));
    return launch_layernorm_fwd(e->hp_ln, E, e->P + e->p2c_lnw, e->P + e->p2c_lnb, nullptr, 0, out, E, e->hp_mean, e->hp_rstd, B, E, s);
  }
  if (c.norm_clips) {
    COATI_TRY(launch_layernorm_fwd(e->hpoint, H, e->P + e->p2c_lnw, e->P + e->p2c_lnb, nullptr, 0, e->hp_ln, H, e->hp_mean, e->hp_rstd, B, H, s));
    x = e->hp_ln;
  }
  return launch_sgemm(x, H, 1, e->P + e->p2c_w, 1, H, out, E, B, E, H, e->P + e->p2c_b, 1.f, 0, s);
}
int smiles_head_fwd(coati_engine* e, float* out, hipStream_t s) {
  const coati_config& c = e->cfg;
  const int C = c.n_hidden_xformer, E = c.n_embd_common, B = e->B;
  const float* x = e->hstop;
  if (c.norm_clips && c.old_architecture) {
    COATI_TRY(launch_sgemm(x, C, 1, e->P + e->s2c_w, 1, C, e->hs_ln, E, B, E, C, e->P + e->s2c_b, 1.f, 0, s));
    return launch_layernorm_fwd(e->hs_ln, E, e->P + e->s2c_lnw, e->P + e->s2c_lnb, nullptr, 0, out, E, e->hs_mean, e->hs_rstd, B, E, s);
  }
  if (c.norm_clips) {
    COATI_TRY(launch_layernorm_fwd(e->hstop, C, e->P + e->s2c_lnw, e->P + e->s2c_lnb, nullptr, 0, e->hs_ln, C, e->hs_mean, e->hs_rstd, B, C, s));
    x = e->hs_ln;
  }
  return launch_sgemm(x, C, 1, e->P + e->s2c_w, 1, C, out, E, B, E, C, e->P + e->s2c_b, 1.f, 0, s);
}

int coati2_head_fwd(coati_engine* e, const coati_engine::Coati2Head& h, const float* x, float* out, int B, hipStream_t s) {
  const int C = e->cfg.n_hidden_xformer, E = e->cfg.n_embd_common;
  const float* P = e->P;
  COATI_TRY(launch_layernorm_fwd(x, C, P + h.lnw, P + h.lnb, nullptr, 0, e->hs_ln, C, e->hs_mean, e->hs_rstd, B, C, s));
  COATI_TRY(launch_sgemm(e->hs_ln, C, 1, P + h.w1, 1, C, e->c2_u, 2 * E, B, 2 * E, C, P + h.b1, 1.f, 0, s));
  COATI_TRY(launch_swiglu(e->c2_u, 2 * E, e->sa, E, B, E, s));
  COATI_TRY(launch_sgemm(e->sa, E, 1, P + h.w2, 1, E, out, E, B, E, E, P + h.b2, 1.f, 0, s));
  if (h.residual) COATI_TRY(launch_axpy(x, out, 1.f, (long long)B * E, s));
  return COATI_OK;
}

int begin_call(coati_engine* e, const char* entry, void* workspace, int64_t workspace_bytes, int B, int T1, int T2, int A, float* scal) {
  Arena ar{reinterpret_cast<char*>(workspace), 0, (size_t)workspace_bytes, false};
  const size_t need = carve(e, ar, B, T1, T2, A, B);
  COATI_CHECK_ARG((int64_t)need <= workspace_bytes, "%s: workspace too small (%zu > %lld)", entry, need, (long long)workspace_bytes);
  if (e->nce) e->nce_cap = ((size_t)workspace_bytes - (size_t)(reinterpret_cast<char*>(e->nce) - reinterpret_cast<char*>(workspace))) / sizeof(float);
  e->B = B; e->T1 = T1; e->T2 = T2; e->A = A;
  if (scal) e->scal = scal;
  e->have_fwd = false;
  e->decoder_pending = false;
  e->have_ws = true;
  return COATI_OK;
}
int clear_errors(coati_engine* e, float* scal, hipStream_t s) {
  if (scal) HIPCHK(hipMemsetAsync(scal, 0, 16 * sizeof(float), s));
  HIPCHK(hipMemsetAsync(e->err_flag, 0, 4 * sizeof(int), s));
  return COATI_OK;
}
int publish_errors(coati_engine* e, float* scal, hipStream_t s) {
  HIPCHK(hipMemcpyAsync(scal + 6, e->err_flag, sizeof(int), hipMemcpyDeviceToDevice, s));
  return COATI_OK;
}

int pack_pass(coati_engine* e, XPass& p, const long long* targets, int64_t rows, hipStream_t s) {
  COATI_TRY(launch_seq_pack(p.idx, targets, e->cfg.pad_token, p.B, p.T, (int)rows, p.off, p.row_src, p.row_t, targets ? p.ypk : nullptr, e->err_flag, s, p.ord));
  p.packed = true;
  p.M = (int)rows;
  return COATI_OK;
}

int stop_rows_head_fwd(coati_engine* e, float* out, hipStream_t s) {
  const XPass& p = e->p1;
  const int C = e->cfg.n_hidden_xformer;
  if (p.tail) HIPCHK(hipMemcpyAsync(e->hstop, p.t_xf, (size_t)p.B * C * sizeof(float), hipMemcpyDeviceToDevice, s));
  else COATI_TRY(launch_gather_rows(p.xf32, e->stop_pos, e->hstop, p.B, p.T, C, s, p.packed ? p.off : nullptr));
  if (e->enc_to_coati > 0) return coati2_head_fwd(e, e->c2s, e->hstop, out, p.B, s);
  return smiles_head_fwd(e, out, s);
}
int token_tower_fwd(coati_engine* e, float* out, hipStream_t s) {
  COATI_TRY(launch_find_stop(e->p1.idx, e->cfg.stop_token, e->stop_pos, e->err_flag, e->p1.B, e->p1.T, s));
  COATI_TRY(xformer_fwd(e, e->p1, nullptr, s));
  return stop_rows_head_fwd(e, out, s);
}

int special_token_add(coati_engine* e, SgemmBatch& sb, const float* h, float* act, float* tok, const float** out, hipStream_t s) {
  const int E = e->cfg.n_embd_common, B = e->B;
  *out = h;
  if (!e->cfg.token_mlp) return COATI_OK;
  COATI_TRY(launch_silu_fwd(h, act, (long long)B * E, s));
  COATI_TRY(sgemm_batch_add(sb, act, E, 1, e->P + e->tokw, 1, E, tok, E, B, E, E, e->P + e->tokb, 1.f, 0));
  *out = tok;
  return COATI_OK;
}

int last_row_logits(coati_engine* e, const float* x, long long ldx, float* logits, int64_t ldl, hipStream_t s) {
  auto& d = e->dec;
  const int C = e->cfg.n_hidden_xformer;
  COATI_TRY(launch_layernorm_fwd(x, ldx, e->P + e->lnfw, e->P + e->lnfb, d.af, C, nullptr, 0, d.mean, d.rstd, d.B, C, s));
  return gemm(e, SITE_NONE, d.af, 0, C, e->S + e->lmhead, C, d.B, e->cfg.n_tok, C, logits, ldl, nullptr, EPI_F32, nullptr, nullptr, 0, s);
}
int pass_logits(coati_engine* e, int site, float* logits, int64_t ldl, hipStream_t s) {
  const int C = e->cfg.n_hidden_xformer;
  return gemm(e, site, e->p2.af, 0, C, e->S + e->lmhead, C, e->B * e->T2, e->cfg.n_tok, C, logits, ldl, nullptr, EPI_F32, nullptr, nullptr, 0, s);
}

}

extern "C" {

int coati_engine_create(const coati_config* cfg, coati_engine** out) {
  COATI_CHECK_ARG(cfg && out, "engine_create: null argument");
  const int C = cfg->n_hidden_xformer, H = cfg->n_hidden_e3nn, E = cfg->n_embd_common;
  COATI_CHECK_SHAPE(cfg->n_head > 0 && (C == cfg->n_head * 16 || C == cfg->n_head * 32), "engine_create: head size must be 16 or 32 (C=%d, n_head=%d)", C, cfg->n_head);
  COATI_CHECK_SHAPE(C % 64 == 0 && H % 64 == 0 && C <= 1024 && H <= 1024, "engine_create: C=%d and H=%d must be multiples of 64 (<=1024)", C, H);
  COATI_CHECK_SHAPE(E == C, "engine_create: n_embd_common (%d) must equal n_hidden_xformer (%d)", E, C);
  COATI_CHECK_SHAPE(cfg->n_seq > 0 && cfg->n_seq <= 256 && cfg->n_tok > 8, "engine_create: n_seq must be <= 256");
  COATI_CHECK_SHAPE(cfg->n_layer_xformer >= 1 && cfg->n_layer_e3gnn >= 0, "engine_create: bad layer counts");
  COATI_CHECK_SHAPE(!cfg->use_fp8 || C % 128 == 0, "engine_create: fp8 mode needs n_hidden_xformer %% 128 == 0 (C=%d)", C);
  COATI_CHECK_ARG(!(cfg->residual && cfg->torch_emb), "engine_create: residual and torch_emb together size the node MLPs for 28 one-hot features and feed them H embedding columns (the reference fails in its first forward: e3gnn_clip.py:100, e_gcl_sparse.py:289)");
  COATI_CHECK_SHAPE(!(cfg->old_architecture && cfg->norm_clips) || H == E, "engine_create: old_architecture needs n_hidden_e3nn == n_embd_common (%d, %d): point_to_clip's LayerNorm is sized by the one and applied to the other (clip_e2e.py:410-413)", H, E);
  coati_engine* e = new coati_engine();
  e->cfg = *cfg;
  build_layout(e);
  *out = e;
  return COATI_OK;
}

int coati_engine_create_coati2(const coati_config* cfg, int enc_to_coati, coati_engine** out) {
  COATI_CHECK_ARG(cfg && out, "engine_create_coati2: null argument");
  COATI_CHECK_ARG(enc_to_coati >= 0 && enc_to_coati <= 2, "engine_create_coati2: enc_to_coati must be 0 (linear), 1 (swiglu_mlp) or 2 (swiglu_resnet), not %d",
                  enc_to_coati);
  COATI_CHECK_ARG(!cfg->use_point_encoder, "engine_create_coati2: COATI2 has no point encoder (use_point_encoder must be 0)");
  COATI_CHECK_ARG(!cfg->use_fp8, "engine_create_coati2: fp8 is not available for COATI2");
  COATI_CHECK_ARG(!cfg->norm_embed, "engine_create_coati2: the COATI2 transformer has no norm_embed");
  const int C = cfg->n_hidden_xformer, E = cfg->n_embd_common;
  COATI_CHECK_SHAPE(E == C, "engine_create_coati2: embed_dim (%d) must equal n_hidden_xformer (%d)", E, C);
  coati_config c = *cfg;
  c.n_layer_e3gnn = 0;
  c.n_hidden_e3nn = C;
  c.norm_clips = 1;
  c.token_mlp = 0;
  c.torch_emb = 0;
  c.old_architecture = 0;
  c.residual = 0;
  COATI_CHECK_SHAPE(c.n_head > 0 && (C == c.n_head * 16 || C == c.n_head * 32), "engine_create_coati2: head size must be 16 or 32 (C=%d, n_head=%d)", C, c.n_head);
  COATI_CHECK_SHAPE(C % 64 == 0 && C <= 1024, "engine_create_coati2: n_hidden_xformer=%d must be a multiple of 64 (<=1024)", C);
  COATI_CHECK_SHAPE(c.n_seq > 0 && c.n_seq <= 256 && c.n_tok > 8, "engine_create_coati2: n_seq must be <= 256");
  COATI_CHECK_SHAPE(c.n_layer_xformer >= 1, "engine_create_coati2: bad layer count");
  coati_engine* e = new coati_engine();
  e->cfg = c;
  e->enc_to_coati = enc_to_coati;
  build_layout(e);
  *out = e;
  return COATI_OK;
}

void coati_engine_destroy(coati_engine* e) {
  if (!e) return;
  for (auto& g : e->dec.graph)
    if (g) hipGraphExecDestroy(g);
  for (auto ev : e->ev) hipEventDestroy(ev);
  if (e->ev_fork) hipEventDestroy(e->ev_fork);
  if (e->ev_join) hipEventDestroy(e->ev_join);
  if (e->side) hipStreamDestroy(e->side);
  for (int i = 0; i < 6; ++i) {
    if (e->h_tab_ev[i]) hipEventDestroy(e->h_tab_ev[i]);
    if (e->h_tab[i]) hipHostFree(e->h_tab[i]);
  }
  delete e;
}

int64_t coati_engine_param_elems(const coati_engine* e) { return e ? e->n_params : 0; }
int64_t coati_engine_trainable_elems(const coati_engine* e) { return e ? e->n_trainable : 0; }
int coati_engine_n_entries(const coati_engine* e) { return e ? (int)e->entries.size() : 0; }
int coati_engine_entry(const coati_engine* e, int i, char* name, int name_cap, int64_t* offset, int32_t* rows, int32_t* cols) {
  COATI_CHECK_ARG(e && i >= 0 && i < (int)e->entries.size() && name && name_cap > 0, "engine_entry: bad argument");
  const Entry& en = e->entries[i];
  snprintf(name, name_cap, "%s", en.name.c_str());
  if (offset) *offset = en.off;
  if (rows) *rows = en.rows;
  if (cols) *cols = en.cols;
  return COATI_OK;
}
int64_t coati_engine_shadow_elems(const coati_engine* e) { return e ? e->n_shadow : 0; }

int coati_engine_reserve(coati_engine* e, int B, int T1, int T2, int A) {
  COATI_CHECK_ARG(e && B >= 0 && T1 >= 0 && T2 >= 0 && A >= 0, "engine_reserve: bad argument");
  COATI_CHECK_SHAPE(T1 <= e->cfg.n_seq && T2 <= e->cfg.n_seq, "engine_reserve: T1=%d T2=%d beyond n_seq=%d", T1, T2, e->cfg.n_seq);
  if (B > e->cap_B) e->cap_B = B;
  if (T1 > e->cap_T1) e->cap_T1 = T1;
  if (T2 > e->cap_T2) e->cap_T2 = T2;
  if (A > e->cap_A) e->cap_A = A;
  return COATI_OK;
}

int64_t coati_engine_workspace_bytes(const coati_engine* e, int B, int T1, int T2, int A, int Bg) {
  if (!e || B <= 0 || T1 <= 0 || T2 <= 0 || A <= 0) return 0;
  coati_engine tmp = *e;
  tmp.ev.clear();
  Arena ar{nullptr, 0, 0, true};
  return (int64_t)carve(&tmp, ar, B, T1, T2, A, Bg);
}

int coati_engine_bind(coati_engine* e, float* params, float* grads, float* adam_m, float* adam_v, uint16_t* shadow,
                      const float* rope_cos, const float* rope_sin, const int32_t* lut_ix, const int32_t* lut_iy) {
  COATI_CHECK_ARG(e && params && shadow && rope_cos && rope_sin && lut_ix && lut_iy, "engine_bind: null argument");
  e->P = params; e->G = grads; e->Mo = adam_m; e->Vo = adam_v; e->S = shadow;
  e->cos_t = rope_cos; e->sin_t = rope_sin; e->lut_ix = lut_ix; e->lut_iy = lut_iy;
  return COATI_OK;
}

int64_t coati_engine_fp8_bytes(const coati_engine* e) { return e ? e->n_fp8 : 0; }
int coati_engine_bind_fp8(coati_engine* e, uint8_t* fp8_shadow, int64_t bytes) {
  COATI_CHECK_ARG(e && e->cfg.use_fp8 && fp8_shadow && bytes >= e->n_fp8, "engine_bind_fp8: not an fp8 engine / buffer too small");
  e->S8 = fp8_shadow;
  return COATI_OK;
}

static int refresh_fp8_weights(coati_engine* e, hipStream_t s) {
  if (!e->cfg.use_fp8) return COATI_OK;
  COATI_CHECK_ARG(e->S8, "fp8 mode: coati_engine_bind_fp8 has not been called");
  const int C = e->cfg.n_hidden_xformer;
  for (const XLayerP& w : e->xl) {
    const int64_t src[8] = {w.attnw, w.projw, w.fc1w, w.fc2w, w.attnT, w.projT, w.fc1T, w.fc2T};
    const int rows[8] = {3 * C, C, 4 * C, C, C, C, C, 4 * C}, cols[8] = {C, C, C, 4 * C, 3 * C, C, 4 * C, C};
    for (int i = 0; i < 8; ++i)
      COATI_TRY(launch_quant_mx8(e->S + src[i], 0, cols[i], e->S8 + w.q8[i], cols[i], e->S8 + w.s8[i], rows[i], cols[i], s));
  }
  return COATI_OK;
}

static int refresh_shadows_impl(coati_engine* e, void* stream, bool natural_done) {
  COATI_CHECK_ARG(e && e->P && e->S, "refresh_shadows: engine not bound");
  hipStream_t s = (hipStream_t)stream;
  ProfScope ps(e, SITE_OPTIM, 0, s);
  if (!natural_done) COATI_TRY(launch_cast_bf16(e->P, e->S, e->n_params, s));
  if (e->d_jobs != nullptr) {
    if (!e->jobs_uploaded) {
      if (hipMemcpyAsync(e->d_jobs, e->jobs.data(), e->jobs.size() * sizeof(ShadowJob), hipMemcpyHostToDevice, s) != hipSuccess ||
          hipMemcpyAsync(e->d_tile_start, e->tile_start.data(), e->tile_start.size() * sizeof(int), hipMemcpyHostToDevice, s) != hipSuccess) {
        coati_set_error("refresh_shadows: job table upload failed");
        return COATI_EHIP;
      }
      e->jobs_uploaded = true;
    }
    COATI_TRY(launch_shadow_jobs(e->d_jobs, e->d_tile_start, (int)e->jobs.size(), e->n_job_tiles, e->P, e->S, s));
    return refresh_fp8_weights(e, s);
  }
  for (const ShadowJob& j : e->jobs) {
    if (j.transpose) COATI_TRY(launch_transpose_cast(e->P + j.src_off, j.ld_src, e->S + j.dst_off, j.ld_dst, j.rows, j.cols, s));
    else COATI_TRY(launch_pack_rows_cast(e->P + j.src_off, j.ld_src, e->S + j.dst_off, j.ld_dst, j.rows, j.cols, s));
  }
  return refresh_fp8_weights(e, s);
}

int coati_engine_refresh_shadows(coati_engine* e, void* stream) { return refresh_shadows_impl(e, stream, false); }

static int lmhead_ce_partial(coati_engine* e, hipStream_t s, int* tiles_v) {
  const coati_config& c = e->cfg;
  const int C = c.n_hidden_xformer, M2 = e->p2.M;
  GemmArgs a;
  memset(&a, 0, sizeof(a));
// ... 735 lines not shown
```

coati_amd/csrc/kernels.h:

```cpp
#pragma once
#include "common.h"

enum CoatiEpi {
  EPI_BF16 = 0,
  EPI_F32 = 1,
  EPI_RES_F32 = 2,
  EPI_GELU = 3,
  EPI_DGELU = 4,
  EPI_SILU = 5,
  EPI_DSILU = 6,
  EPI_ACC_F32 = 7,
  EPI_CE_PARTIAL = 8,
  EPI_CE_BWD = 9,
  EPI_EDGE_DPRE = 10,
  EPI_QKV_ROPE = 11,
  EPI_GELU_GRAD = 12,
  EPI_MUL_AUX = 13,
  EPI_LNBWD = 14,
  EPI_CE_BWD_ROW = 15,
  EPI_COUNT = 16
};

struct GemmArgs {
  const int* m_dev;
  const void* A;
  long long lda;
  const bf16_t* B;
  long long ldb;
  int M, N, K;
  void* C;
  long long ldc;
  int n_store;
  const float* bias;
  const void* aux_in;
  void* aux_out;
  long long ld_aux;
  const float* lse;
  const long long* target;
  const float* scal;
  float2* partial;
  int partial_tile;
  const bf16_t* P;
  long long ldp;
  const float* d2;
  const float* w1c;
  long long w1c_stride;
  const float* b1;
  int natom;
  int H;
  const int* e_bj;
  const int* e_bk;
  const float* rope_cos;
  const float* rope_sin;
  int rope_T;
  int rope_C;
  int rope_hs;
  const int* rope_pos;
  const int* rope_row_t;
  unsigned char* q8_out;
  unsigned char* q8_scales;
  long long ld_q8;
  const float* ln_x;
  long long ln_ldx;
  const float* ln_gamma;
  const float* ln_beta;
  float* ln_mean;
  float* ln_rstd;
  const float* lnb_x;
  long long lnb_ldx;
  const float* lnb_mean;
  const float* lnb_rstd;
  const float* lnb_gamma;
  float* lnb_partial;
  const bf16_t* chain_W;
  long long chain_ldw;
  bf16_t* chain_C;
  long long chain_ldc;
  const float* row_scale;
};

int launch_gemm_nt(const GemmArgs& a, int a_f32, int epi, hipStream_t s);
bool gemm_rb256_supported(const GemmArgs& a, int a_f32, int epi);
bool gemm_ring_lnbwd_supported(const GemmArgs& a, int* nwg);
bool gemm_rb256_ln_fusable(const GemmArgs& a, int epi);
int gemm_ce_tile_width(const GemmArgs& a);
int launch_gemm_rb256(const GemmArgs& a, int epi, hipStream_t s);
bool gemm_rb16_supported(const GemmArgs& a, int a_f32, int epi);
bool gemm_rb16_resident_supported(const GemmArgs& a, int a_f32, int epi);
int launch_gemm_rb16_resident(const GemmArgs& a, int epi, hipStream_t s);
int launch_gemm_rb16(const GemmArgs& a, int epi, hipStream_t s);
#ifdef COATI_EXPERIMENTAL
struct Mlp64Args {
  const float* x;
  long long ldx;
  const float* gamma;
  const float* beta;
  bf16_t* a2;
  float* mean;
  float* rstd;
  const bf16_t* W1;
  const float* b1;
  const bf16_t* W2;
  const float* b2;
  bf16_t* g;
  unsigned char* codes;
  float* out;
  long long ldo;
  int M;
};
bool mlp64_fwd_supported(int M, int C, int hidden);
int launch_mlp64_fwd(const Mlp64Args& a, hipStream_t s);
bool gemm_t32_supported(const GemmArgs& a, int a_f32, int epi);
int launch_gemm_t32(const GemmArgs& a, int epi, hipStream_t s);
#endif
bool gemm_ring256_supported(const GemmArgs& a, int a_f32, int epi);
int launch_gemm_ring256(const GemmArgs& a, int epi, hipStream_t s);
int launch_gemm_mx8(const GemmArgs& a, const unsigned char* sa, const unsigned char* sb, int epi, hipStream_t s);
int launch_quant_mx8(const void* x, int x_f32, long long ldx, unsigned char* q, long long ldq, unsigned char* scales, int M, int K, hipStream_t s);

struct WgradArgs {
  const void* A;
  long long lda;
  const bf16_t* B;
  long long ldb;
  int M, N, K;
  float* dW;
  long long ldw;
  float* dbias;
  int n_out;
  const int* m_dev = nullptr;
};
int launch_wgrad(const WgradArgs& a, int a_f32, hipStream_t s);
struct WgradTile {
  WgradArgs p;
  int tiles_k;
  int tile;
  int c_begin = 0, c_end = 0;
};
int launch_wgrad_table(const WgradTile* dev_table, int n_tiles, hipStream_t s, int tile_size = 128, int M_rt = 0);
bool wgrad_table_tile256_ok(const WgradArgs& a);
int launch_wgrad_split_table(const WgradTile* dev_table, int n_entries, hipStream_t s);
#ifdef __cplusplus
#include <vector>
int wgrad_table_append(std::vector<WgradTile>& tab, const WgradArgs& a, int tile_size = 128);
int wgrad_table_append_split(std::vector<WgradTile>& tab, const WgradArgs& a, int n_splits);
#endif

#define SGEMM_BATCH_MAX 6
struct SgemmProb {
  const float *A, *B, *bias;
  float* C;
  long long ars, acs, brs, bcs, ldc;
  int M, N, K, accumulate, ksplit, tx, ty, tz, wg0;
  float alpha;
};
struct SgemmBatch {
  int n = 0;
  SgemmProb p[SGEMM_BATCH_MAX];
};
int sgemm_batch_add(SgemmBatch& b, const float* A, long long ars, long long acs, const float* B, long long brs, long long bcs,
                    float* C, long long ldc, int M, int N, int K, const float* bias, float alpha, int accumulate);
int launch_sgemm_batch(const SgemmBatch& b, hipStream_t s);
int launch_sgemm(const float* A, long long ars, long long acs, const float* B, long long brs, long long bcs,
                 float* C, long long ldc, int M, int N, int K, const float* bias, float alpha, int accumulate,
                 hipStream_t s);

int launch_layernorm_fwd(const float* x, long long ldx, const float* gamma, const float* beta, bf16_t* y16,
                         long long ld16, float* y32, long long ld32, float* mean, float* rstd, int M, int C,
                         hipStream_t s);
int launch_layernorm_bwd(const void* dy, int dy_f32, long long lddy, const float* x, long long ldx, int x_is_xhat,
                         const float* mean, const float* rstd, const float* gamma, const float* dres,
                         float* dx, bf16_t* dx16, float* dgamma, float* dbeta, float* partial, int M, int C, hipStream_t s);
int launch_layernorm_bwd_deferred(const void* dy, int dy_f32, long long lddy, const float* x, long long ldx, int x_is_xhat,
                                  const float* mean, const float* rstd, const float* gamma, const float* dres, float* dx,
                                  bf16_t* dx16, float* partial, int* nblk_out, int M, int C, hipStream_t s);
#define COATI_LN_MAX_SLOTS 72
struct LnFinishBatch {
  int n;
  long long dg_off[COATI_LN_MAX_SLOTS];
  long long db_off[COATI_LN_MAX_SLOTS];
  int nblk[COATI_LN_MAX_SLOTS];
};
int launch_ln_finish_batched(const float* partial, long long slot_stride, int nblk, float* grad_base, const LnFinishBatch& b,
                             int C, hipStream_t s);
#define COATI_LN_PARTIAL_ROWS 2048

int launch_attn_fwd(const bf16_t* qkv, bf16_t* y, float* lse, int B, int T, int n_head, int head_size, hipStream_t s,
                    const int* seq_off = nullptr, const int* seq_ord = nullptr);
int launch_attn_bwd(const bf16_t* qkv, const bf16_t* y, const bf16_t* dy, const float* lse, float* dscratch, bf16_t* dqkv,
                    const float* cos, const float* sin, int B, int T, int n_head, int head_size, hipStream_t s,
                    const int* seq_off = nullptr, const int* seq_ord = nullptr);
int launch_attn16_fwd(const bf16_t* qkv, bf16_t* y, float* lse, int B, int T, int n_head, hipStream_t s, const int* seq_off, const int* seq_ord = nullptr);
int launch_attn16_bwd(const bf16_t* qkv, const bf16_t* y, const bf16_t* dy, const float* lse, bf16_t* dqkv, const float* cos_t,
                      const float* sin_t, int B, int T, int n_head, hipStream_t s, const int* seq_off, const int* seq_ord = nullptr);

#ifdef COATI_EXPERIMENTAL
struct AttnBlockArgs {
  const float* x;
  float* xmid;
  const float* ln_g;
  const float* ln_b;
  float* mean;
  float* rstd;
  bf16_t* a1;
  const bf16_t* Wqkv;
  const float* bqkv;
  const bf16_t* Wproj;
  const float* bproj;
  bf16_t* qkv;
  bf16_t* y;
  float* lse;
  const float* cos_t;
  const float* sin_t;
  const int* row_src;
  const int* grp;
  int Tl, M;
};
bool attn_block_fwd_supported(int B, int T, int C, int n_head);
int launch_attn_groups(const int* seq_off, int B, int T, int* grp, hipStream_t s);
int launch_attn_block_fwd(const AttnBlockArgs& a, hipStream_t s);
int launch_ab_probe_swap(unsigned* out, hipStream_t s);
#endif

int launch_embed_fwd(const long long* idx, const float* table, const float* injection, int unk_token, float* x,
                     int B, int T, int C, int V, hipStream_t s, const int* row_src = nullptr, int rows = 0, int mode = 0);
int launch_embed_bwd(const long long* idx, const float* dx, float* dtable, float* dinjection, int unk_token,
                     int B, int T, int C, int V, hipStream_t s, const int* off = nullptr, int inj_only = 0);
int launch_seq_pack(const long long* tok, const long long* y, int pad_token, int B, int T, int rows_expect, int* off,
                    int* row_src, int* row_t, long long* ypk, int* err, hipStream_t s, int* ord = nullptr);
int launch_seq_pack_len(const int* len, int B, int T, int rows_expect, int* off, int* row_src, int* row_t, int* err, hipStream_t s,
                        int* ord = nullptr);
int launch_find_stop(const long long* idx, int stop_token, int* pos, int* err, int B, int T, hipStream_t s);
int launch_gather_rows(const float* x, const int* pos, float* out, int B, int T, int C, hipStream_t s, const int* off = nullptr);
int launch_scatter_rows_add(const float* dout, const int* pos, float* dx, int B, int T, int C, hipStream_t s, const int* off = nullptr);
int launch_scatter_rows_bf16(const bf16_t* src, const int* pos, bf16_t* dst, int B, int T, int C, hipStream_t s, const int* off = nullptr);
int launch_bad_rows(const long long* tokens, unsigned char* bad, int B, int T, hipStream_t s);
int launch_attn_decode(const bf16_t* qkv, bf16_t* cache, bf16_t* y, int B, int n_head, int head_size, int Tmax, int pos,
                       const int* pos_dev, hipStream_t s);
int launch_add_int(int* x, int v, int set, hipStream_t s);
int launch_attn_decode_rows(const bf16_t* qkv, bf16_t* cache, bf16_t* y, int B, int n_head, int head_size, int Tmax, const int* pos,
                            hipStream_t s);
int launch_decode_rows_prep(const int* pos, const int* inj_len, const long long* tokens, int* rope_t, long long* tok_inj, int B, int Tmax,
                            hipStream_t s);
int launch_topk_sample(const float* logits, long long ldl, int B, int V, int k, float inv_temp, const float* u,
                       long long* tok_out, int* stopped, int stop_token, int pad_token, hipStream_t s);
int launch_topk_sample_prompt(const float* logits, long long ldl, int B, int V, int k, float inv_temp, const float* u,
                              const long long* prompt, long long ldp, const int* plen, int pos, long long* tok_out, int* stopped,
                              int stop_token, int pad_token, hipStream_t s);
int launch_topk_sample_rows(const float* logits, long long ldl, int B, int V, int k, float inv_temp, const float* u, long long ldu,
                            const long long* prompt, long long ldp, const int* plen, const int* req, int* pos, long long* out,
                            long long ldo, long long* tok_next, int* done, int Tmax, int stop_token, hipStream_t s);
int launch_kv_cache_fill_rows(const bf16_t* qkv, bf16_t* cache, const int* row_src, int R, int B, int T, int n_head, int head_size,
                              int Tmax, hipStream_t s);
int launch_gather_last_rows(const float* x, const int* off, float* out, int B, int C, int R, hipStream_t s);
int launch_kv_cache_fill(const bf16_t* qkv, bf16_t* cache, int B, int m, int n_head, int head_size, int Tmax, hipStream_t s);
int launch_batch_ncols(const long long* tok, int B, int S, int* ncols, hipStream_t s);
int launch_batch_tail(const long long* tok, int B, int S, int ncol, long long* tok_out, long long* y_out,
                      const long long* masked, int n_masked, hipStream_t s);

int launch_ce_finish(const float2* partial, int tiles_n, const bf16_t* a, long long lda, const bf16_t* W,
                     long long ldw, const long long* target, float* lse, float* scal, int M, int C, int V,
                     hipStream_t s);
int launch_ce_seq(const float2* partial, int tiles_n, const bf16_t* a, long long lda, const bf16_t* W, long long ldw,
                  const long long* target, const int* off, float* nll, int B, int T, int C, int V, hipStream_t s);
int launch_ce_seq_bwd(const float2* partial, int tiles_n, const bf16_t* a, long long lda, const bf16_t* W, long long ldw,
                      const long long* target, const int* off, const float* weights, float* nll, float* lse, float* row_scale, int B, int T,
                      int C, int V, hipStream_t s);

int launch_gnn_embed(const long long* atoms, const int* lut_ix, const int* lut_iy, const float* W, const float* b,
                     float* h32, bf16_t* h16, long long ld16, float* rstd, float* mask, int BA, int H,
                     hipStream_t s, int* err = nullptr);
int launch_gnn_node_res_silu(const float* u32, const long long* atoms, const int* lut_ix, const int* lut_iy, const float* W3c, long long ldw,
                             bf16_t* upre, bf16_t* t16, int BA, int H, hipStream_t s);
int launch_gnn_onehot_wgrad(const long long* atoms, const int* lut_ix, const int* lut_iy, const bf16_t* du, float* dW, long long ldw, int BA,
                            int H, hipStream_t s);
int launch_gnn_embed_bwd(const long long* atoms, const int* lut_ix, const int* lut_iy, const float* de,
                         float* dW, float* db, int BA, int H, hipStream_t s);
int launch_gnn_geom(const float* coords, const float* mask, float cutoff, float* d2, float* w, int B, int A,
                    hipStream_t s);
int launch_gnn_compact(const float* w_dense, const float* d2_dense, int* seg, int* n_edges, int* e_bj, int* e_bk, int* e_rev,
                       float* e_d2, float* e_w, int* pos, int B, int A, hipStream_t s);
int launch_gnn_edge_pre_c(const bf16_t* P, long long ldp, const int* seg, const int* e_bk, const float* e_d2, const float* w1c,
                          long long w1c_stride, const float* b1, bf16_t* e1, int BA, int H, hipStream_t s);
int launch_gnn_edge_reduce_c(const bf16_t* s2, const int* seg, const float* e_w, bf16_t* mi, long long ldmi, int BA, int H, hipStream_t s);
int launch_gnn_edge_fwd_fused(const bf16_t* P, long long ldp, const int* seg, const int* e_bk, const float* e_d2, const float* e_w,
                              const float* w1c, long long w1c_stride, const float* b1, const bf16_t* W3, long long ldw, const float* b3,
                              bf16_t* e1, bf16_t* s2, bf16_t* mi, long long ldmi, int BA, int H, hipStream_t s);
int launch_gnn_edge_reduce_bwd_c(const bf16_t* dmi, long long lddmi, const bf16_t* s2, const int* seg, const float* e_w,
                                 bf16_t* ds2, int BA, int H, hipStream_t s);
int launch_gnn_edge_pre_bwd_c(const bf16_t* dpre, const int* seg, const int* e_rev, const float* e_d2, bf16_t* dP, long long lddp,
                              float* dw1c, long long dw1c_stride, float* db1, int BA, int H, hipStream_t s);
int launch_gnn_readout(const float* o, const float* mask, float* hp, int B, int A, int H, hipStream_t s);
int launch_gnn_readout_bwd(const float* dhp, const float* mask, bf16_t* dout, int B, int A, int H, hipStream_t s);

int launch_silu_fwd(const float* x, float* y, long long n, hipStream_t s);
int launch_silu_bwd(const float* x, const float* dy, float* dx, long long n, int accumulate, hipStream_t s);
int launch_swiglu(const float* u, long long ldu, float* g, long long ldg, int B, int N, hipStream_t s);
int launch_group_mean_rows(const float* x, long long ldx, const int* off, const float* w, const float* fallback, float* out, int G, int E,
                           hipStream_t s);
int launch_select_rows(const unsigned char* use_a, const float* a, const float* b, float* out, int B, int C,
                       hipStream_t s);
int launch_select_rows_bwd(const unsigned char* use_a, const float* dout, float* da, float* db, int B, int C,
                           hipStream_t s);
int launch_axpy(const float* x, float* y, float alpha, long long n, hipStream_t s);
int launch_infonce_rows2(float* logits, float* logits2, long long ld, int R, int N, int label0, const unsigned char* bad,
                         float* loss_sum, float* loss_sum2, const float* inv_count, float gscale, hipStream_t s);
int launch_infonce_rows(float* logits, long long ld, int R, int N, int label0, const unsigned char* bad,
                        float* loss_sum, const float* inv_count, float gscale, hipStream_t s);
int launch_count_valid(const unsigned char* bad, int n, float* out_count, float* out_inv, hipStream_t s);
int launch_colsum2(const float* a, const float* b2, const unsigned char* bad, float* out, int B, int E, hipStream_t s);
int launch_center_rows(const float* z, const unsigned char* bad, const float* sum, const float* count, float* zc, int B, int E, hipStream_t s);
int launch_standardize(const float* z, const unsigned char* bad, const float* stats, const float* count, float* zt, float* rsigma,
                       int B, int E, hipStream_t s);
int launch_barlow_dc(float* C, const float* count, float lam, float* loss, int E, hipStream_t s);
int launch_standardize_bwd(const float* dzt, const float* zt, const unsigned char* bad, const float* rsigma, const float* m,
                           const float* count, float scale, float* dz, int B, int E, hipStream_t s);

int launch_grad_sqnorm(const float* g, long long n, float* partial, int n_partial, float* out_norm, float max_norm,
                       float* out_coef, hipStream_t s);
int launch_adamw(float* p, const float* g, float* m, float* v, bf16_t* shadow, long long n, float lr, float b1,
                 float b2, float eps, float wd, int step, const float* coef, float gscale, hipStream_t s, const int* skip = nullptr);
int launch_cast_bf16(const float* src, bf16_t* dst, long long n, hipStream_t s);
int launch_transpose_cast(const float* src, long long ld_src, bf16_t* dst, long long ld_dst, int rows, int cols,
                          hipStream_t s);
int launch_pack_rows_cast(const float* src, long long ld_src, bf16_t* dst, long long ld_dst, int rows, int cols,
                          hipStream_t s);

struct ShadowJob {
  long long src_off, dst_off;
  int ld_src, ld_dst, rows, cols, transpose;
};
int launch_shadow_jobs(const ShadowJob* jobs, const int* tile_start, int n_jobs, int n_tiles, const float* P, bf16_t* S,
                       hipStream_t s);
```

Before: 50160 molecules/s.

## Fuse E3GNN node-MLP GEMM chains with layernorm into single row-block kernels

```diff
diff --git a/coati_amd/build.py b/coati_amd/build.py
--- a/coati_amd/build.py
+++ b/coati_amd/build.py
@@ -8,7 +8,7 @@
 LIBDIR = os.path.join(HERE, "lib")
 LIB = os.path.join(LIBDIR, "libcoati_hip_x.so" if os.environ.get("COATI_AMD_EXPERIMENTAL") == "1" else "libcoati_hip.so")
 OBJDIR = os.path.join(HERE, "build")
-HIP_UNITS = ["gemm.hip", "gemm_rb.hip", "gemm_rb16.hip", "gemm_ring.hip", "gemm_mx8.hip", "norm.hip", "attention.hip", "attention16.hip", "embed.hip", "gnn.hip", "loss.hip", "optim.hip", "batch.hip", "decode.hip"]
+HIP_UNITS = ["gemm.hip", "gemm_rb.hip", "gemm_rb16.hip", "gemm_ring.hip", "gemm_mx8.hip", "norm.hip", "attention.hip", "attention16.hip", "embed.hip", "gnn.hip", "gnn_chain.hip", "loss.hip", "optim.hip", "batch.hip", "decode.hip"]
 CPP_UNITS = ["engine.cpp", "capi.cpp", "tokenizer.cpp", "comm.cpp"]
 FLAGS = ["--offload-arch=gfx950", "-O3", "-std=c++17", "-fPIC", "-Wno-unused-value", "-mllvm", "-amdgpu-mfma-vgpr-form=1"] + os.environ.get("COATI_AMD_CXXFLAGS", "").split()
 
diff --git a/coati_amd/csrc/engine.cpp b/coati_amd/csrc/engine.cpp
--- a/coati_amd/csrc/engine.cpp
+++ b/coati_amd/csrc/engine.cpp
@@ -555,6 +555,10 @@
   static const bool on = []() { const char* v = getenv("COATI_GNN_EDGE_FUSED"); return !(v && v[0] == '0'); }();
   return on;
 }
+static bool gnn_chain_on(const coati_config& c) {
+  static const bool on = []() { const char* v = getenv("COATI_GNN_CHAIN"); return !(v && v[0] == '0'); }();
+  return on && c.n_hidden_e3nn == 256 && !c.residual && c.n_layer_e3gnn > 0;
+}
 static bool lpt_on() {
   static const bool on = []() { const char* v = getenv("COATI_ATTN_LPT"); return !(v && v[0] == '0'); }();
   return on;
@@ -1097,8 +1101,20 @@
     COATI_TRY(launch_gnn_geom(coords, e->g_mask, c.msg_cutoff, e->g_d2, e->g_w, B, A, s));
     COATI_TRY(launch_gnn_compact(e->g_w, e->g_d2, e->g_seg, e->g_ne, e->g_ebj, e->g_ebk, e->g_erev, e->g_ed2, e->g_ew, e->g_pos, B, A, s));
   }
+  const bool chain = gnn_chain_on(c);
+  const double pb_n0 = (double)BA * 2 * H * 2 + 2.0 * H * H * 2 + (double)BA * H * 4, pb_sq = (double)BA * H * 2 + (double)H * H * 2;
+  const double fl_sq = 2.0 * BA * H * H;
   for (int l = 0; l < Lg; ++l) {
     const GLayerP& w = e->gl[l];
+    if (chain) {
+      if (l == 0) {
+        GnnChainFwd a;
+        memset(&a, 0, sizeof(a));
+        a.M = BA; a.H = H; a.X = e->g_hcat[0]; a.ldx = 2 * H; a.w1ab = e->S + w.w1ab; a.P = e->g_P[0]; a.ldp = 2 * H;
+        ProfScope ps(e, SITE_GNN_NODE_GEMM, 2.0 * fl_sq, s, pb_sq + (double)H * H * 2 + (double)BA * 2 * H * 2);
+        COATI_TRY(launch_gnn_chain_fwd(a, 0, s));
+      }
+    } else
     COATI_TRY(gemm(e, SITE_GNN_NODE_GEMM, e->g_hcat[l], 0, 2 * H, e->S + w.w1ab, H, BA, 2 * H, H, e->g_P[l], 2 * H, nullptr, EPI_BF16, nullptr, nullptr, 0, s));
     if (H == 256 && gnn_edge_fused_on()) {
       ProfScope ps(e, SITE_GNN_EDGE_GEMM, 0, s, (double)BA * (H * 2 + 4 + H * 2) + (double)H * H * 2, (double)H * 2 + 12 + (double)H * 4, 2.0 * H * H + 6.0 * H);
@@ -1122,6 +1138,22 @@
       COATI_TRY(launch_gnn_edge_reduce_c(e->g_s2[l], e->g_seg, e->g_ew, e->g_hcat[l] + H, 2 * H, BA, H, s));
     }
     }
+    if (chain) {
+      const bool last = (l + 1 == Lg);
+      GnnChainFwd a;
+      memset(&a, 0, sizeof(a));
+      a.M = BA; a.H = H; a.X = e->g_hcat[l]; a.ldx = 2 * H;
+      a.n0w = e->S + w.n0w; a.n0b = e->P + w.n0b; a.upre = e->g_upre[l]; a.t = e->g_t[l];
+      a.n3w = e->S + w.n3w; a.n3b = e->P + w.n3b; a.hres = e->g_h32[l];
+      a.hout32 = e->g_h32[l + 1]; a.rstd = e->g_rstd[l + 1]; a.h16 = last ? e->g_hfin16 : e->g_hcat[l + 1]; a.ld16 = last ? H : 2 * H;
+      if (!last) { a.w1ab = e->S + e->gl[l + 1].w1ab; a.P = e->g_P[l + 1]; a.ldp = 2 * H; }
+      else { a.d0w = e->S + e->gd0w; a.d0b = e->P + e->gd0b; a.dpre = e->g_dpre; a.td = e->g_td; a.d3w = e->S + e->gd3w; a.d3b = e->P + e->gd3b; a.o2 = e->g_o2; }
+      const double bytes = pb_n0 + (double)H * H * 2 + (double)BA * H * 4 + (double)BA * (H * 6 + 4) +
+                           (last ? 2.0 * H * H * 2 + (double)BA * H * (4 + 4) : 2.0 * H * H * 2 + (double)BA * 2 * H * 2);
+      ProfScope ps(e, SITE_GNN_NODE_GEMM, 5.0 * fl_sq, s, bytes);
+      COATI_TRY(launch_gnn_chain_fwd(a, last ? 2 : 1, s));
+      continue;
+    }
     if (c.residual) {
       COATI_TRY(gemm(e, SITE_GNN_NODE_GEMM, e->g_hcat[l], 0, 2 * H, e->S + w.n0p, 2 * H, BA, H, 2 * H, e->g_o, H, e->P + w.n0b, EPI_F32, nullptr, nullptr, 0, s));
       ProfScope ps(e, SITE_GNN_ELEMWISE, 0, s, (double)BA * (H * 4 + 8 + H * 4));
@@ -1136,8 +1168,10 @@
       COATI_TRY(launch_layernorm_fwd(e->g_o, H, nullptr, nullptr, last ? e->g_hfin16 : e->g_hcat[l + 1], last ? H : 2 * H, e->g_h32[l + 1], H, nullptr, e->g_rstd[l + 1], BA, H, s));
     }
   }
+  if (!chain) {
   COATI_TRY(gemm(e, SITE_GNN_NODE_GEMM, e->g_hfin16, 0, H, e->S + e->gd0w, H, BA, H, H, e->g_td, H, e->P + e->gd0b, EPI_SILU, nullptr, e->g_dpre, H, s));
   COATI_TRY(gemm(e, SITE_GNN_NODE_GEMM, e->g_td, 0, H, e->S + e->gd3w, H, BA, H, H, e->g_o2, H, e->P + e->gd3b, EPI_F32, nullptr, nullptr, 0, s));
+  }
   ProfScope ps(e, SITE_GNN_ELEMWISE, 0, s, (double)BA * (H * 4 + 4) + (double)B * H * 4);
   return launch_gnn_readout(e->g_o2, e->g_mask, e->hpoint, B, A, H, s);
 }
@@ -1177,27 +1211,50 @@
   const int H = c.n_hidden_e3nn, Lg = c.n_layer_e3gnn, B = e->B, A = e->A, BA = B * A, Me = BA * A;
   float *DH = e->g_DH, *DO = e->g_DO;
   const bool grp = e->gnn_wg_group;
+  const bool chain = gnn_chain_on(c);
+  const double pb_sq = (double)BA * H * 2 + (double)H * H * 2, fl_sq = 2.0 * BA * H * H;
+  auto chain_tail = [&](GnnChainBwd& a, int l) {
+    const GLayerP& w = e->gl[l];
+    a.M = BA; a.H = H; a.A = A;
+    a.xhat = e->g_h32[l + 1]; a.rstd = e->g_rstd[l + 1]; a.DO = DO;
+    a.DO16 = grp ? e->gl_DO16[l] : e->g_DO16; a.n3T = e->S + w.n3T; a.upre = e->g_upre[l]; a.du = grp ? e->gl_du[l] : e->g_du;
+    a.n0T = e->S + w.n0T; a.dmi = e->g_dmi;
+  };
+  const double tail_bytes = (double)BA * (H * 4 + 4 + H * 2) + (double)BA * H * 4 + (double)BA * H * (4 + 2) + 3.0 * H * H * 2;
+  if (chain) {
+    GnnChainBwd a;
+    memset(&a, 0, sizeof(a));
+    a.dhp = dhpoint; a.mask = e->g_mask; a.do2 = e->g_do2; a.d3T = e->S + e->gd3T; a.dpre = e->g_dpre; a.dtd = e->g_dtd; a.d0T = e->S + e->gd0T;
+    chain_tail(a, Lg - 1);
+    {
+      ProfScope ps(e, SITE_GNN_NODE_GEMM, 5.0 * fl_sq, s, (double)B * H * 4 + (double)BA * (4 + H * 2) + (double)BA * H * 4 + 2.0 * H * H * 2 + tail_bytes);
+      COATI_TRY(launch_gnn_chain_bwd(a, 0, 0, s));
+    }
+  } else {
   {
     ProfScope ps(e, SITE_GNN_ELEMWISE, 0, s, (double)B * H * 4 + (double)BA * (H * 2 + 4));
     COATI_TRY(launch_gnn_readout_bwd(dhpoint, e->g_mask, e->g_do2, B, A, H, s));
   }
   COATI_TRY(gemm(e, SITE_GNN_NODE_GEMM, e->g_do2, 0, H, e->S + e->gd3T, H, BA, H, H, e->g_dtd, H, nullptr, EPI_DSILU, e->g_dpre, nullptr, H, s));
+  }
   if (!grp) COATI_TRY(wgrad(e, SITE_GNN_WGRAD, e->g_do2, 0, H, e->g_td, H, BA, H, H, e->G + e->gd3w, H, e->G + e->gd3b, 0, s));
-  COATI_TRY(gemm(e, SITE_GNN_NODE_GEMM, e->g_dtd, 0, H, e->S + e->gd0T, H, BA, H, H, DH, H, nullptr, EPI_F32, nullptr, nullptr, 0, s));
+  if (!chain) COATI_TRY(gemm(e, SITE_GNN_NODE_GEMM, e->g_dtd, 0, H, e->S + e->gd0T, H, BA, H, H, DH, H, nullptr, EPI_F32, nullptr, nullptr, 0, s));
   if (!grp) COATI_TRY(wgrad(e, SITE_GNN_WGRAD, e->g_dtd, 0, H, e->g_hfin16, H, BA, H, H, e->G + e->gd0w, H, e->G + e->gd0b, 0, s));
   for (int l = Lg - 1; l >= 0; --l) {
     const GLayerP& w = e->gl[l];
     bf16_t* const DO16 = grp ? e->gl_DO16[l] : e->g_DO16;
     bf16_t* const du = grp ? e->gl_du[l] : e->g_du;
     bf16_t* const dP = grp ? e->gl_dP[l] : e->g_dP;
-    {
+    if (!chain) {
       ProfScope ps(e, SITE_GNN_ELEMWISE, 0, s, (double)BA * (H * 4 + H * 4 + 4 + H * 4 + H * 2));
       COATI_TRY(launch_layernorm_bwd(DH, 1, H, e->g_h32[l + 1], H, 1, nullptr, e->g_rstd[l + 1], nullptr, nullptr, DO, DO16, nullptr, nullptr, e->ln_partial, BA, H, s));
     }
-    COATI_TRY(gemm(e, SITE_GNN_NODE_GEMM, DO16, 0, H, e->S + w.n3T, H, BA, H, H, du, H, nullptr, EPI_DSILU, e->g_upre[l], nullptr, H, s));
+    if (!chain) COATI_TRY(gemm(e, SITE_GNN_NODE_GEMM, DO16, 0, H, e->S + w.n3T, H, BA, H, H, du, H, nullptr, EPI_DSILU, e->g_upre[l], nullptr, H, s));
     if (!grp) COATI_TRY(wgrad(e, SITE_GNN_WGRAD, DO16, 0, H, e->g_t[l], H, BA, H, H, e->G + w.n3w, H, e->G + w.n3b, 0, s));
+    if (!chain) {
     COATI_TRY(gemm(e, SITE_GNN_NODE_GEMM, du, 0, H, e->S + w.n0T, H, BA, H, H, DO, H, nullptr, EPI_ACC_F32, nullptr, nullptr, 0, s));
     COATI_TRY(gemm(e, SITE_GNN_NODE_GEMM, du, 0, H, e->S + w.n0T + (int64_t)H * H, H, BA, H, H, e->g_dmi, H, nullptr, EPI_BF16, nullptr, nullptr, 0, s));
+    }
     if (!grp) COATI_TRY(wgrad(e, SITE_GNN_WGRAD, du, 0, H, e->g_hcat[l], 2 * H, BA, H, 2 * H, e->G + w.n0w, 2 * H + (c.residual ? 28 : 0), e->G + w.n0b, 0, s));
     if (c.residual) {
       ProfScope ps(e, SITE_GNN_ELEMWISE, 0, s, (double)BA * (H * 2 + 8));
@@ -1228,6 +1285,24 @@
       ProfScope ps(e, SITE_GNN_ELEMWISE, 0, s, (double)BA * (H * 4 + 4), (double)H * 4 + 8, 4.0 * H);
       COATI_TRY(launch_gnn_edge_pre_bwd_c(e->g_dpre1, e->g_seg, e->g_erev, e->g_ed2, dP, 2 * H, e->G + w.e0w + 2 * H, 2 * H + 1, e->G + w.e0b, BA, H, s));
     }
+    if (chain) {
+      GnnChainBwd a;
+      memset(&a, 0, sizeof(a));
+      a.dP = dP; a.lddp = 2 * H; a.w1abT = e->S + w.w1abT; a.DOin = DO;
+      const double head_bytes = (double)BA * 2 * H * 2 + 2.0 * H * H * 2 + (double)BA * H * 4;
+      if (l > 0) {
+        float* const DOsave = DO;
+        DO = DH;
+        chain_tail(a, l - 1);
+        DO = DOsave;
+        ProfScope ps(e, SITE_GNN_NODE_GEMM, 6.0 * fl_sq, s, head_bytes + tail_bytes);
+        COATI_TRY(launch_gnn_chain_bwd(a, 1, 0, s));
+      } else {
+        a.M = BA; a.H = H; a.A = A; a.xhat = e->g_h32[0]; a.rstd = e->g_rstd[0]; a.DO = DH;
+        ProfScope ps(e, SITE_GNN_NODE_GEMM, 2.0 * fl_sq, s, head_bytes + (double)BA * (H * 4 + 4 + H * 4));
+        COATI_TRY(launch_gnn_chain_bwd(a, 1, 1, s));
+      }
+    } else
     COATI_TRY(gemm(e, SITE_GNN_NODE_GEMM, dP, 0, 2 * H, e->S + w.w1abT, 2 * H, BA, H, 2 * H, DO, H, nullptr, EPI_ACC_F32, nullptr, nullptr, 0, s));
     if (!grp) {
       COATI_TRY(wgrad(e, SITE_GNN_WGRAD, dP, 0, 2 * H, e->g_hcat[l], 2 * H, BA, H, H, e->G + w.e0w, 2 * H + 1, nullptr, 0, s));
@@ -1237,8 +1312,8 @@
   }
   if (grp) COATI_TRY(gnn_wgrad_group(e, s));
   {
-    ProfScope ps(e, SITE_GNN_ELEMWISE, 0, s, (double)BA * (H * 4 + H * 4 + 4 + H * 4) + (double)BA * (8 + H * 4) + 30.0 * H * 4);
-    COATI_TRY(launch_layernorm_bwd(DH, 1, H, e->g_h32[0], H, 1, nullptr, e->g_rstd[0], nullptr, nullptr, DO, nullptr, nullptr, nullptr, e->ln_partial, BA, H, s));
+    ProfScope ps(e, SITE_GNN_ELEMWISE, 0, s, (chain ? 0.0 : (double)BA * (H * 4 + H * 4 + 4 + H * 4)) + (double)BA * (8 + H * 4) + 30.0 * H * 4);
+    if (!chain) COATI_TRY(launch_layernorm_bwd(DH, 1, H, e->g_h32[0], H, 1, nullptr, e->g_rstd[0], nullptr, nullptr, DO, nullptr, nullptr, nullptr, e->ln_partial, BA, H, s));
     if (e->cfg.torch_emb) COATI_TRY(launch_gnn_embed_bwd(e->atoms, nullptr, nullptr, DO, e->G + e->gembw, nullptr, BA, H, s));
     else COATI_TRY(launch_gnn_embed_bwd(e->atoms, e->lut_ix, e->lut_iy, DO, e->G + e->gembw, e->G + e->gembb, BA, H, s));
   }
diff --git a/coati_amd/csrc/gnn_chain.hip b/coati_amd/csrc/gnn_chain.hip
--- /dev/null
+++ b/coati_amd/csrc/gnn_chain.hip
@@ -0,0 +1,554 @@
+#include <cstdlib>
+#include <cstring>
+#include "kernels.h"
+
+#define GC_K 256
+#define GC_BN 64
+#define GC_TILE_HALFS (GC_BN * GC_K)
+#define GC_MAXT 24
+#define GC_NBUF 2
+#define GC_EPS 1e-5f
+
+typedef float gc_f32x4 __attribute__((ext_vector_type(4)));
+typedef __attribute__((address_space(3))) void gc_lds_void;
+typedef __attribute__((address_space(1))) const void gc_gbl_void;
+
+struct GcTile {
+  const bf16_t* src;
+  long long ldb;
+};
+
+__device__ __forceinline__ int gc_wrow(int a, int i) { return 32 * (a >> 1) + 8 * (i >> 2) + 4 * (a & 1) + (i & 3); }
+__device__ __forceinline__ int gc_swz(int n) { return (n & 3) | (((n >> 3) & 3) << 2) | (((n >> 2) & 1) << 4); }
+
+struct GcLane {
+  int wave, lane, fr, kq;
+  int wofs[4], wsw[4];
+  int colA, colB;
+};
+
+template <int W>
+__device__ __forceinline__ void gc_load_tile(const GcTile& t, bf16_t* S, const GcLane& L) {
+#pragma unroll
+  for (int i = 0; i < 32 / W; ++i) {
+    const int k = L.wave + W * i;
+    const int r = 2 * k + (L.lane >> 5), q = L.lane & 31;
+    const bf16_t* src = t.src + (long long)r * t.ldb + ((q ^ gc_swz(r)) * 8);
+    __builtin_amdgcn_global_load_lds((gc_gbl_void*)src, (gc_lds_void*)(S + k * 512), 16, 0, 0);
+  }
+}
+
+template <int W, int NT>
+__device__ __forceinline__ void gc_mma(const GcTile* tiles, int t, const bf16_t* __restrict__ cur, bf16_t* __restrict__ nxt,
+                                       const bf16x8 (&af)[8], gc_f32x4 (&acc)[4], const GcLane& L) {
+  if (t + GC_NBUF - 1 < NT) gc_load_tile<W>(tiles[t + GC_NBUF - 1], nxt, L);
+  bf16x8 wf[2][4];
+#pragma unroll
+  for (int a = 0; a < 4; ++a) wf[0][a] = *reinterpret_cast<const bf16x8*>(cur + L.wofs[a] + ((L.kq ^ L.wsw[a]) * 8));
+#pragma unroll
+  for (int ks = 0; ks < 8; ++ks) {
+    if (ks + 1 < 8) {
+#pragma unroll
+      for (int a = 0; a < 4; ++a) wf[(ks + 1) & 1][a] = *reinterpret_cast<const bf16x8*>(cur + L.wofs[a] + (((4 * (ks + 1) + L.kq) ^ L.wsw[a]) * 8));
+    }
+#pragma unroll
+    for (int a = 0; a < 4; ++a) acc[a] = __builtin_amdgcn_mfma_f32_16x16x32_bf16(wf[ks & 1][a], af[ks], acc[a], 0, 0, 0);
+    __builtin_amdgcn_sched_barrier(0);
+  }
+  constexpr int PER = 32 / W;
+  const int ahead = (t + GC_NBUF - 1 < NT ? t + GC_NBUF - 1 : NT - 1) - (t + 1);
+  if (ahead >= 2) __builtin_amdgcn_s_waitcnt(0x0f70 | ((2 * PER) & 15) | (((2 * PER) >> 4) << 14));
+  else if (ahead == 1) __builtin_amdgcn_s_waitcnt(0x0f70 | (PER & 15) | ((PER >> 4) << 14));
+  else __builtin_amdgcn_s_waitcnt(0x0f70);
+  __syncthreads();
+}
+
+#define GC_CUR(t) (Bs + ((t) % GC_NBUF) * GC_TILE_HALFS)
+#define GC_NXT(t) (Bs + (((t) + GC_NBUF - 1) % GC_NBUF) * GC_TILE_HALFS)
+template <int W, int NT>
+__device__ __forceinline__ void gc_prime(const GcTile* tiles, bf16_t* Bs, const GcLane& L) {
+#pragma unroll
+  for (int t = 0; t < GC_NBUF - 1 && t < NT; ++t) gc_load_tile<W>(tiles[t], Bs + t * GC_TILE_HALFS, L);
+}
+
+__device__ __forceinline__ void gc_zero(gc_f32x4 (&acc)[4]) {
+#pragma unroll
+  for (int a = 0; a < 4; ++a) acc[a] = gc_f32x4{0.f, 0.f, 0.f, 0.f};
+}
+__device__ __forceinline__ void gc_out(const gc_f32x4 (&acc)[4], const float* bias, int c0, int c1, float (&v0)[8], float (&v1)[8]) {
+#pragma unroll
+  for (int r = 0; r < 4; ++r) { v0[r] = acc[0][r]; v0[4 + r] = acc[1][r]; v1[r] = acc[2][r]; v1[4 + r] = acc[3][r]; }
+  if (bias != nullptr) {
+    const float4 a0 = *reinterpret_cast<const float4*>(bias + c0), a1 = *reinterpret_cast<const float4*>(bias + c0 + 4);
+    const float4 b0 = *reinterpret_cast<const float4*>(bias + c1), b1 = *reinterpret_cast<const float4*>(bias + c1 + 4);
+    v0[0] += a0.x; v0[1] += a0.y; v0[2] += a0.z; v0[3] += a0.w; v0[4] += a1.x; v0[5] += a1.y; v0[6] += a1.z; v0[7] += a1.w;
+    v1[0] += b0.x; v1[1] += b0.y; v1[2] += b0.z; v1[3] += b0.w; v1[4] += b1.x; v1[5] += b1.y; v1[6] += b1.z; v1[7] += b1.w;
+  }
+}
+__device__ __forceinline__ void gc_ld8(const float* p, float (&v)[8]) {
+  const float4 a = *reinterpret_cast<const float4*>(p), b = *reinterpret_cast<const float4*>(p + 4);
+  v[0] = a.x; v[1] = a.y; v[2] = a.z; v[3] = a.w; v[4] = b.x; v[5] = b.y; v[6] = b.z; v[7] = b.w;
+}
+__device__ __forceinline__ void gc_st8(float* p, const float (&v)[8]) {
+  *reinterpret_cast<float4*>(p) = make_float4(v[0], v[1], v[2], v[3]);
+  *reinterpret_cast<float4*>(p + 4) = make_float4(v[4], v[5], v[6], v[7]);
+}
+__device__ __forceinline__ GcLane gc_lane() {
+  GcLane L;
+  L.lane = threadIdx.x & 63;
+  L.wave = __builtin_amdgcn_readfirstlane(threadIdx.x >> 6);
+  L.fr = L.lane & 15;
+  L.kq = L.lane >> 4;
+#pragma unroll
+  for (int a = 0; a < 4; ++a) {
+    const int n = gc_wrow(a, L.fr);
+    L.wofs[a] = n * GC_K;
+    L.wsw[a] = gc_swz(n);
+  }
+  L.colA = 8 * L.kq;
+  L.colB = 32 + 8 * L.kq;
+  return L;
+}
+__device__ __forceinline__ uint4 gc_silu_store(float (&v)[8], bf16_t* pre, bf16_t* out, bool ok) {
+  const uint4 up = pack8(v);
+  float o[8];
+#pragma unroll
+  for (int e = 0; e < 8; ++e) o[e] = silu_f(v[e]);
+  const uint4 u = pack8(o);
+  if (ok) {
+    *reinterpret_cast<uint4*>(pre) = up;
+    *reinterpret_cast<uint4*>(out) = u;
+  }
+  return u;
+}
+__device__ __forceinline__ uint4 gc_dsilu_store(const float (&v)[8], const uint4& pre, bf16_t* out, bool ok) {
+  float x[8], o[8];
+  unpack8(pre, x);
+#pragma unroll
+  for (int e = 0; e < 8; ++e) o[e] = v[e] * dsilu_f(x[e]);
+  const uint4 u = pack8(o);
+  if (ok) *reinterpret_cast<uint4*>(out) = u;
+  return u;
+}
+
+struct GcFwdArgs {
+  GcTile tile[GC_MAXT];
+  int ntile, M;
+  const bf16_t* X; long long ldx;
+  const float* n0b; bf16_t* upre; bf16_t* t;
+  const float* n3b; const float* hres;
+  float* hout32; float* rstd; bf16_t* h16; long long ld16;
+  bf16_t* P; long long ldp;
+  const float* d0b; bf16_t* dpre; bf16_t* td; const float* d3b; float* o2;
+};
+
+template <int MODE, int W>
+__global__ __launch_bounds__(64 * W) void gnn_chain_fwd_kernel(GcFwdArgs p) {
+  extern __shared__ __attribute__((aligned(16))) unsigned char smem[];
+  bf16_t* const Bs = reinterpret_cast<bf16_t*>(smem);
+  constexpr int NT = MODE == 0 ? 8 : 20;
+  float* const BiasS = reinterpret_cast<float*>(smem + (size_t)GC_NBUF * GC_TILE_HALFS * 2);
+  if constexpr (MODE != 0) {
+    for (int c = threadIdx.x; c < GC_K; c += 64 * W) {
+      BiasS[c] = p.n0b[c];
+      BiasS[GC_K + c] = p.n3b[c];
+      if constexpr (MODE == 2) { BiasS[2 * GC_K + c] = p.d0b[c]; BiasS[3 * GC_K + c] = p.d3b[c]; }
+    }
+  }
+  const GcLane L = gc_lane();
+  const int row = (blockIdx.x * W + L.wave) * 16 + L.fr;
+  const bool ok = row < p.M;
+  const long long rc = ok ? row : p.M - 1;
+  gc_prime<W, NT>(p.tile, Bs, L);
+
+  bf16x8 haf[8];
+  {
+    const bf16_t* xp = p.X + rc * p.ldx + L.kq * 8;
+#pragma unroll
+    for (int ks = 0; ks < 8; ++ks) haf[ks] = *reinterpret_cast<const bf16x8*>(xp + ks * 32);
+  }
+  __builtin_amdgcn_s_waitcnt(0x0f70);
+  __syncthreads();
+  int t = 0;
+  gc_f32x4 acc[4];
+  float v0[8], v1[8];
+
+  if constexpr (MODE != 0) {
+    bf16x8 maf[8], taf[8];
+    {
+      const bf16_t* xp = p.X + rc * p.ldx + GC_K + L.kq * 8;
+#pragma unroll
+      for (int ks = 0; ks < 8; ++ks) maf[ks] = *reinterpret_cast<const bf16x8*>(xp + ks * 32);
+    }
+#pragma unroll
+    for (int jt = 0; jt < 4; ++jt) {
+      gc_zero(acc);
+      gc_mma<W, NT>(p.tile, t, GC_CUR(t), GC_NXT(t), haf, acc, L); ++t;
+      gc_mma<W, NT>(p.tile, t, GC_CUR(t), GC_NXT(t), maf, acc, L); ++t;
+      const int c0 = jt * GC_BN + L.colA, c1 = jt * GC_BN + L.colB;
+      gc_out(acc, BiasS, c0, c1, v0, v1);
+      const uint4 u0 = gc_silu_store(v0, p.upre + rc * GC_K + c0, p.t + rc * GC_K + c0, ok);
+      const uint4 u1 = gc_silu_store(v1, p.upre + rc * GC_K + c1, p.t + rc * GC_K + c1, ok);
+      taf[2 * jt] = __builtin_bit_cast(bf16x8, u0);
+      taf[2 * jt + 1] = __builtin_bit_cast(bf16x8, u1);
+    }
+    float o[4][16];
+#pragma unroll
+    for (int jt = 0; jt < 4; ++jt) {
+      const int c0 = jt * GC_BN + L.colA, c1 = jt * GC_BN + L.colB;
+      float r0[8], r1[8];
+      gc_ld8(p.hres + rc * GC_K + c0, r0);
+      gc_ld8(p.hres + rc * GC_K + c1, r1);
+      gc_zero(acc);
+      gc_mma<W, NT>(p.tile, t, GC_CUR(t), GC_NXT(t), taf, acc, L); ++t;
+      gc_out(acc, BiasS + GC_K, c0, c1, v0, v1);
+#pragma unroll
+      for (int e = 0; e < 8; ++e) { o[jt][e] = v0[e] + r0[e]; o[jt][8 + e] = v1[e] + r1[e]; }
+    }
+    float sm = 0.f;
+#pragma unroll
+    for (int jt = 0; jt < 4; ++jt)
+#pragma unroll
+      for (int e = 0; e < 16; ++e) sm += o[jt][e];
+    sm += __shfl_xor(sm, 16, 64);
+    sm += __shfl_xor(sm, 32, 64);
+    const float mean = sm / (float)GC_K;
+    float q = 0.f;
+#pragma unroll
+    for (int jt = 0; jt < 4; ++jt)
+#pragma unroll
+      for (int e = 0; e < 16; ++e) { const float d = o[jt][e] - mean; q += d * d; }
+    q += __shfl_xor(q, 16, 64);
+    q += __shfl_xor(q, 32, 64);
+    const float rstd = 1.0f / sqrtf(q / (float)GC_K + GC_EPS);
+    if (ok && L.kq == 0) p.rstd[row] = rstd;
+#pragma unroll
+    for (int jt = 0; jt < 4; ++jt) {
+      const int c0 = jt * GC_BN + L.colA, c1 = jt * GC_BN + L.colB;
+#pragma unroll
+      for (int e = 0; e < 8; ++e) { v0[e] = (o[jt][e] - mean) * rstd; v1[e] = (o[jt][8 + e] - mean) * rstd; }
+      const uint4 u0 = pack8(v0), u1 = pack8(v1);
+      if (ok) {
+        gc_st8(p.hout32 + rc * GC_K + c0, v0);
+        gc_st8(p.hout32 + rc * GC_K + c1, v1);
+        *reinterpret_cast<uint4*>(p.h16 + rc * p.ld16 + c0) = u0;
+        *reinterpret_cast<uint4*>(p.h16 + rc * p.ld16 + c1) = u1;
+      }
+      haf[2 * jt] = __builtin_bit_cast(bf16x8, u0);
+      haf[2 * jt + 1] = __builtin_bit_cast(bf16x8, u1);
+    }
+  }
+
+  if constexpr (MODE != 2) {
+#pragma unroll
+    for (int jt = 0; jt < 8; ++jt) {
+      gc_zero(acc);
+      gc_mma<W, NT>(p.tile, t, GC_CUR(t), GC_NXT(t), haf, acc, L); ++t;
+      const int c0 = jt * GC_BN + L.colA, c1 = jt * GC_BN + L.colB;
+      gc_out(acc, nullptr, c0, c1, v0, v1);
+      if (ok) {
+        *reinterpret_cast<uint4*>(p.P + rc * p.ldp + c0) = pack8(v0);
+        *reinterpret_cast<uint4*>(p.P + rc * p.ldp + c1) = pack8(v1);
+      }
+    }
+  } else {
+    bf16x8 taf[8];
+#pragma unroll
+    for (int jt = 0; jt < 4; ++jt) {
+      gc_zero(acc);
+      gc_mma<W, NT>(p.tile, t, GC_CUR(t), GC_NXT(t), haf, acc, L); ++t;
+      const int c0 = jt * GC_BN + L.colA, c1 = jt * GC_BN + L.colB;
+      gc_out(acc, BiasS + 2 * GC_K, c0, c1, v0, v1);
+      const uint4 u0 = gc_silu_store(v0, p.dpre + rc * GC_K + c0, p.td + rc * GC_K + c0, ok);
+      const uint4 u1 = gc_silu_store(v1, p.dpre + rc * GC_K + c1, p.td + rc * GC_K + c1, ok);
+      taf[2 * jt] = __builtin_bit_cast(bf16x8, u0);
+      taf[2 * jt + 1] = __builtin_bit_cast(bf16x8, u1);
+    }
+#pragma unroll
+    for (int jt = 0; jt < 4; ++jt) {
+      gc_zero(acc);
+      gc_mma<W, NT>(p.tile, t, GC_CUR(t), GC_NXT(t), taf, acc, L); ++t;
+      const int c0 = jt * GC_BN + L.colA, c1 = jt * GC_BN + L.colB;
+      gc_out(acc, BiasS + 3 * GC_K, c0, c1, v0, v1);
+      if (ok) {
+        gc_st8(p.o2 + rc * GC_K + c0, v0);
+        gc_st8(p.o2 + rc * GC_K + c1, v1);
+      }
+    }
+  }
+}
+
+struct GcBwdArgs {
+  GcTile tile[GC_MAXT];
+  int ntile, M, A;
+  const float* dhp; const float* mask; bf16_t* do2; const bf16_t* dpre; bf16_t* dtd;
+  const bf16_t* dP; long long lddp; const float* DOin;
+  const float* xhat; const float* rstd;
+  float* DO; bf16_t* DO16; const bf16_t* upre; bf16_t* du; bf16_t* dmi;
+};
+
+template <int HEAD, int TAIL, int W>
+__global__ __launch_bounds__(64 * W) void gnn_chain_bwd_kernel(GcBwdArgs p) {
+  extern __shared__ __attribute__((aligned(16))) unsigned char smem[];
+  bf16_t* const Bs = reinterpret_cast<bf16_t*>(smem);
+  constexpr int NT = 8 + (TAIL == 0 ? 12 : 0);
+  const GcLane L = gc_lane();
+  const int row = (blockIdx.x * W + L.wave) * 16 + L.fr;
+  const bool ok = row < p.M;
+  const long long rc = ok ? row : p.M - 1;
+  gc_prime<W, NT>(p.tile, Bs, L);
+
+  int t = 0;
+  gc_f32x4 acc[4];
+  float v0[8], v1[8];
+  float dh[4][16];
+  bf16x8 af[8];
+
+  if constexpr (HEAD == 0) {
+    const long long b = rc / p.A;
+    float n = 0.f;
+    for (int a = 0; a < p.A; ++a) n += p.mask[b * p.A + a];
+    n = fmaxf(n, 1.f);
+    const float mk = p.mask[rc];
+#pragma unroll
+    for (int ks = 0; ks < 8; ++ks) {
+      float g[8];
+      gc_ld8(p.dhp + b * GC_K + ks * 32 + L.kq * 8, g);
+#pragma unroll
+      for (int e = 0; e < 8; ++e) g[e] = (g[e] / n) * mk;
+      const uint4 u = pack8(g);
+      if (ok) *reinterpret_cast<uint4*>(p.do2 + rc * GC_K + ks * 32 + L.kq * 8) = u;
+      af[ks] = __builtin_bit_cast(bf16x8, u);
+    }
+    __builtin_amdgcn_s_waitcnt(0x0f70);
+    __syncthreads();
+    bf16x8 bf[8];
+#pragma unroll
+    for (int jt = 0; jt < 4; ++jt) {
+      const int c0 = jt * GC_BN + L.colA, c1 = jt * GC_BN + L.colB;
+      const uint4 x0 = *reinterpret_cast<const uint4*>(p.dpre + rc * GC_K + c0), x1 = *reinterpret_cast<const uint4*>(p.dpre + rc * GC_K + c1);
+      gc_zero(acc);
+      gc_mma<W, NT>(p.tile, t, GC_CUR(t), GC_NXT(t), af, acc, L); ++t;
+      gc_out(acc, nullptr, c0, c1, v0, v1);
+      bf[2 * jt] = __builtin_bit_cast(bf16x8, gc_dsilu_store(v0, x0, p.dtd + rc * GC_K + c0, ok));
+      bf[2 * jt + 1] = __builtin_bit_cast(bf16x8, gc_dsilu_store(v1, x1, p.dtd + rc * GC_K + c1, ok));
+    }
+#pragma unroll
+    for (int jt = 0; jt < 4; ++jt) {
+      gc_zero(acc);
+      gc_mma<W, NT>(p.tile, t, GC_CUR(t), GC_NXT(t), bf, acc, L); ++t;
+      gc_out(acc, nullptr, 0, 0, v0, v1);
+#pragma unroll
+      for (int e = 0; e < 8; ++e) { dh[jt][e] = v0[e]; dh[jt][8 + e] = v1[e]; }
+    }
+  } else {
+    bf16x8 bf[8];
+    {
+      const bf16_t* xp = p.dP + rc * p.lddp + L.kq * 8;
+#pragma unroll
+      for (int ks = 0; ks < 8; ++ks) { af[ks] = *reinterpret_cast<const bf16x8*>(xp + ks * 32); bf[ks] = *reinterpret_cast<const bf16x8*>(xp + GC_K + ks * 32); }
+    }
+    __builtin_amdgcn_s_waitcnt(0x0f70);
+    __syncthreads();
+#pragma unroll
+    for (int jt = 0; jt < 4; ++jt) {
+      const int c0 = jt * GC_BN + L.colA, c1 = jt * GC_BN + L.colB;
+      float r0[8], r1[8];
+      gc_ld8(p.DOin + rc * GC_K + c0, r0);
+      gc_ld8(p.DOin + rc * GC_K + c1, r1);
+      gc_zero(acc);
+      gc_mma<W, NT>(p.tile, t, GC_CUR(t), GC_NXT(t), af, acc, L); ++t;
+      gc_mma<W, NT>(p.tile, t, GC_CUR(t), GC_NXT(t), bf, acc, L); ++t;
+      gc_out(acc, nullptr, c0, c1, v0, v1);
+#pragma unroll
+      for (int e = 0; e < 8; ++e) { dh[jt][e] = v0[e] + r0[e]; dh[jt][8 + e] = v1[e] + r1[e]; }
+    }
+  }
+
+  {
+    const float rs = p.rstd[rc];
+    float s1 = 0.f, s2 = 0.f;
+    float xh[4][16];
+#pragma unroll
+    for (int jt = 0; jt < 4; ++jt) {
+      float a[8], b[8];
+      gc_ld8(p.xhat + rc * GC_K + jt * GC_BN + L.colA, a);
+      gc_ld8(p.xhat + rc * GC_K + jt * GC_BN + L.colB, b);
+#pragma unroll
+      for (int e = 0; e < 8; ++e) { xh[jt][e] = a[e]; xh[jt][8 + e] = b[e]; }
+    }
+#pragma unroll
+    for (int jt = 0; jt < 4; ++jt)
+#pragma unroll
+      for (int e = 0; e < 16; ++e) { s1 += dh[jt][e]; s2 += dh[jt][e] * xh[jt][e]; }
+    s1 += __shfl_xor(s1, 16, 64);
+    s1 += __shfl_xor(s1, 32, 64);
+    s2 += __shfl_xor(s2, 16, 64);
+    s2 += __shfl_xor(s2, 32, 64);
+    s1 = s1 / (float)GC_K;
+    s2 = s2 / (float)GC_K;
+#pragma unroll
+    for (int jt = 0; jt < 4; ++jt)
+#pragma unroll
+      for (int e = 0; e < 16; ++e) dh[jt][e] = rs * (dh[jt][e] - s1 - xh[jt][e] * s2);
+  }
+  if constexpr (TAIL == 1) {
+    if (ok) {
+#pragma unroll
+      for (int jt = 0; jt < 4; ++jt) {
+#pragma unroll
+        for (int e = 0; e < 8; ++e) { v0[e] = dh[jt][e]; v1[e] = dh[jt][8 + e]; }
+        gc_st8(p.DO + rc * GC_K + jt * GC_BN + L.colA, v0);
+        gc_st8(p.DO + rc * GC_K + jt * GC_BN + L.colB, v1);
+      }
+    }
+  } else {
+#pragma unroll
+    for (int jt = 0; jt < 4; ++jt) {
+      const int c0 = jt * GC_BN + L.colA, c1 = jt * GC_BN + L.colB;
+#pragma unroll
+      for (int e = 0; e < 8; ++e) { v0[e] = dh[jt][e]; v1[e] = dh[jt][8 + e]; }
+      const uint4 u0 = pack8(v0), u1 = pack8(v1);
+      if (ok) {
+        *reinterpret_cast<uint4*>(p.DO16 + rc * GC_K + c0) = u0;
+        *reinterpret_cast<uint4*>(p.DO16 + rc * GC_K + c1) = u1;
+      }
+      af[2 * jt] = __builtin_bit_cast(bf16x8, u0);
+      af[2 * jt + 1] = __builtin_bit_cast(bf16x8, u1);
+    }
+    bf16x8 uf[8];
+#pragma unroll
+    for (int jt = 0; jt < 4; ++jt) {
+      const int c0 = jt * GC_BN + L.colA, c1 = jt * GC_BN + L.colB;
+      const uint4 x0 = *reinterpret_cast<const uint4*>(p.upre + rc * GC_K + c0), x1 = *reinterpret_cast<const uint4*>(p.upre + rc * GC_K + c1);
+      gc_zero(acc);
+      gc_mma<W, NT>(p.tile, t, GC_CUR(t), GC_NXT(t), af, acc, L); ++t;
+      gc_out(acc, nullptr, c0, c1, v0, v1);
+      uf[2 * jt] = __builtin_bit_cast(bf16x8, gc_dsilu_store(v0, x0, p.du + rc * GC_K + c0, ok));
+      uf[2 * jt + 1] = __builtin_bit_cast(bf16x8, gc_dsilu_store(v1, x1, p.du + rc * GC_K + c1, ok));
+    }
+#pragma unroll
+    for (int jt = 0; jt < 4; ++jt) {
+      gc_zero(acc);
+      gc_mma<W, NT>(p.tile, t, GC_CUR(t), GC_NXT(t), uf, acc, L); ++t;
+      const int c0 = jt * GC_BN + L.colA, c1 = jt * GC_BN + L.colB;
+      gc_out(acc, nullptr, c0, c1, v0, v1);
+#pragma unroll
+      for (int e = 0; e < 8; ++e) { v0[e] += dh[jt][e]; v1[e] += dh[jt][8 + e]; }
+      if (ok) {
+        gc_st8(p.DO + rc * GC_K + c0, v0);
+        gc_st8(p.DO + rc * GC_K + c1, v1);
+      }
+    }
+#pragma unroll
+    for (int jt = 0; jt < 4; ++jt) {
+      gc_zero(acc);
+      gc_mma<W, NT>(p.tile, t, GC_CUR(t), GC_NXT(t), uf, acc, L); ++t;
+      const int c0 = jt * GC_BN + L.colA, c1 = jt * GC_BN + L.colB;
+      gc_out(acc, nullptr, c0, c1, v0, v1);
+      if (ok) {
+        *reinterpret_cast<uint4*>(p.dmi + rc * GC_K + c0) = pack8(v0);
+        *reinterpret_cast<uint4*>(p.dmi + rc * GC_K + c1) = pack8(v1);
+      }
+    }
+  }
+}
+
+static int gc_waves() {
+  static const int v = []() { const char* e = getenv("COATI_GNN_CHAIN_W"); const int w = e ? atoi(e) : 4; return (w == 2 || w == 8) ? w : 4; }();
+  return v;
+}
+static int gc_add(GcTile* tile, int& n, const bf16_t* Wt, long long ldb, int N, int nk) {
+  COATI_CHECK_ARG(Wt != nullptr && ldb % 8 == 0 && N % GC_BN == 0, "gnn_chain: bad weight operand");
+  for (int jt = 0; jt < N / GC_BN; ++jt)
+    for (int kh = 0; kh < nk; ++kh) {
+      COATI_CHECK_ARG(n < GC_MAXT, "gnn_chain: tile table overflow");
+      tile[n].src = Wt + (long long)jt * GC_BN * ldb + (long long)kh * GC_K;
+      tile[n].ldb = ldb;
+      ++n;
+    }
+  return COATI_OK;
+}
+template <typename K, typename A>
+static int gc_launch(K kern, bool& attr_set, const A& a, int M, int W, hipStream_t s, const char* name) {
+  constexpr size_t lds = (size_t)GC_NBUF * GC_TILE_HALFS * 2 + (size_t)4 * GC_K * 4;
+  if (!attr_set) {
+    if (hipFuncSetAttribute(reinterpret_cast<const void*>(kern), hipFuncAttributeMaxDynamicSharedMemorySize, (int)lds) != hipSuccess) {
+      coati_set_error("%s: hipFuncSetAttribute failed", name);
+      return COATI_EHIP;
+    }
+    attr_set = true;
+  }
+  hipLaunchKernelGGL(kern, dim3(cdiv(cdiv(M, 16), W)), dim3(64 * W), lds, s, a);
+  COATI_LAUNCH_CHECK(name);
+  return COATI_OK;
+}
+#define GC_DISPATCH_W(KERN, ...)                                                          \
+  do {                                                                                    \
+    static bool set2 = false, set4 = false, set8 = false;                                 \
+    const int W_ = gc_waves();                                                            \
+    if (W_ == 2) return gc_launch(KERN<__VA_ARGS__, 2>, set2, a, a.M, 2, s, #KERN);       \
+    if (W_ == 8) return gc_launch(KERN<__VA_ARGS__, 8>, set8, a, a.M, 8, s, #KERN);       \
+    return gc_launch(KERN<__VA_ARGS__, 4>, set4, a, a.M, 4, s, #KERN);                    \
+  } while (0)
+
+int launch_gnn_chain_fwd(const GnnChainFwd& f, int mode, hipStream_t s) {
+  COATI_CHECK_ARG(mode >= 0 && mode <= 2, "gnn_chain_fwd: mode %d", mode);
+  COATI_CHECK_SHAPE(f.H == GC_K && f.M > 0 && f.ldx % 8 == 0, "gnn_chain_fwd: H = 256 only (H=%d)", f.H);
+  GcFwdArgs a;
+  memset(&a, 0, sizeof(a));
+  a.M = f.M; a.X = f.X; a.ldx = f.ldx;
+  COATI_CHECK_ARG(f.X != nullptr, "gnn_chain_fwd: null operand");
+  if (mode != 0) {
+    COATI_CHECK_ARG(f.n0b && f.upre && f.t && f.n3b && f.hres && f.hout32 && f.rstd && f.h16 && f.ld16 % 8 == 0, "gnn_chain_fwd: null operand");
+    COATI_TRY(gc_add(a.tile, a.ntile, f.n0w, 2 * GC_K, GC_K, 2));
+    COATI_TRY(gc_add(a.tile, a.ntile, f.n3w, GC_K, GC_K, 1));
+    a.n0b = f.n0b; a.upre = f.upre; a.t = f.t; a.n3b = f.n3b; a.hres = f.hres;
+    a.hout32 = f.hout32; a.rstd = f.rstd; a.h16 = f.h16; a.ld16 = f.ld16;
+  }
+  if (mode != 2) {
+    COATI_CHECK_ARG(f.P && f.ldp % 8 == 0, "gnn_chain_fwd: null operand");
+    COATI_TRY(gc_add(a.tile, a.ntile, f.w1ab, GC_K, 2 * GC_K, 1));
+    a.P = f.P; a.ldp = f.ldp;
+  } else {
+    COATI_CHECK_ARG(f.d0b && f.dpre && f.td && f.d3b && f.o2, "gnn_chain_fwd: null operand");
+    COATI_TRY(gc_add(a.tile, a.ntile, f.d0w, GC_K, GC_K, 1));
+    COATI_TRY(gc_add(a.tile, a.ntile, f.d3w, GC_K, GC_K, 1));
+    a.d0b = f.d0b; a.dpre = f.dpre; a.td = f.td; a.d3b = f.d3b; a.o2 = f.o2;
+  }
+  COATI_CHECK_ARG(a.ntile == (mode == 0 ? 8 : 20), "gnn_chain_fwd: %d tiles", a.ntile);
+  if (mode == 0) GC_DISPATCH_W(gnn_chain_fwd_kernel, 0);
+  if (mode == 1) GC_DISPATCH_W(gnn_chain_fwd_kernel, 1);
+  GC_DISPATCH_W(gnn_chain_fwd_kernel, 2);
+}
+
+int launch_gnn_chain_bwd(const GnnChainBwd& f, int head, int tail, hipStream_t s) {
+  COATI_CHECK_ARG((head == 0 || head == 1) && (tail == 0 || tail == 1), "gnn_chain_bwd: head %d tail %d", head, tail);
+  COATI_CHECK_SHAPE(f.H == GC_K && f.M > 0 && f.A > 0, "gnn_chain_bwd: H = 256 only (H=%d)", f.H);
+  GcBwdArgs a;
+  memset(&a, 0, sizeof(a));
+  a.M = f.M; a.A = f.A;
+  if (head == 0) {
+    COATI_CHECK_ARG(f.dhp && f.mask && f.do2 && f.dpre && f.dtd && f.M % f.A == 0, "gnn_chain_bwd: null operand");
+    COATI_TRY(gc_add(a.tile, a.ntile, f.d3T, GC_K, GC_K, 1));
+    COATI_TRY(gc_add(a.tile, a.ntile, f.d0T, GC_K, GC_K, 1));
+    a.dhp = f.dhp; a.mask = f.mask; a.do2 = f.do2; a.dpre = f.dpre; a.dtd = f.dtd;
+  } else {
+    COATI_CHECK_ARG(f.dP && f.lddp % 8 == 0 && f.DOin, "gnn_chain_bwd: null operand");
+    COATI_TRY(gc_add(a.tile, a.ntile, f.w1abT, 2 * GC_K, GC_K, 2));
+    a.dP = f.dP; a.lddp = f.lddp; a.DOin = f.DOin;
+  }
+  COATI_CHECK_ARG(f.xhat && f.rstd && f.DO, "gnn_chain_bwd: null operand");
+  a.xhat = f.xhat; a.rstd = f.rstd; a.DO = f.DO;
+  if (tail == 0) {
+    COATI_CHECK_ARG(f.DO16 && f.upre && f.du && f.dmi, "gnn_chain_bwd: null operand");
+    COATI_TRY(gc_add(a.tile, a.ntile, f.n3T, GC_K, GC_K, 1));
+    COATI_TRY(gc_add(a.tile, a.ntile, f.n0T, GC_K, 2 * GC_K, 1));
+    a.DO16 = f.DO16; a.upre = f.upre; a.du = f.du; a.dmi = f.dmi;
+  }
+  COATI_CHECK_ARG(a.ntile == 8 + (tail == 0 ? 12 : 0), "gnn_chain_bwd: %d tiles", a.ntile);
+  if (head == 0 && tail == 0) GC_DISPATCH_W(gnn_chain_bwd_kernel, 0, 0);
+  if (head == 0 && tail == 1) GC_DISPATCH_W(gnn_chain_bwd_kernel, 0, 1);
+  if (head == 1 && tail == 0) GC_DISPATCH_W(gnn_chain_bwd_kernel, 1, 0);
+  GC_DISPATCH_W(gnn_chain_bwd_kernel, 1, 1);
+}
diff --git a/coati_amd/csrc/kernels.h b/coati_amd/csrc/kernels.h
--- a/coati_amd/csrc/kernels.h
+++ b/coati_amd/csrc/kernels.h
@@ -292,6 +292,25 @@
                               float* dw1c, long long dw1c_stride, float* db1, int BA, int H, hipStream_t s);
 int launch_gnn_readout(const float* o, const float* mask, float* hp, int B, int A, int H, hipStream_t s);
 int launch_gnn_readout_bwd(const float* dhp, const float* mask, bf16_t* dout, int B, int A, int H, hipStream_t s);
+struct GnnChainFwd {
+  int M, H;
+  const bf16_t* X; long long ldx;
+  const bf16_t* n0w; const float* n0b; bf16_t* upre; bf16_t* t;
+  const bf16_t* n3w; const float* n3b; const float* hres;
+  float* hout32; float* rstd; bf16_t* h16; long long ld16;
+  const bf16_t* w1ab; bf16_t* P; long long ldp;
+  const bf16_t* d0w; const float* d0b; bf16_t* dpre; bf16_t* td;
+  const bf16_t* d3w; const float* d3b; float* o2;
+};
+int launch_gnn_chain_fwd(const GnnChainFwd& a, int mode, hipStream_t s);
+struct GnnChainBwd {
+  int M, H, A;
+  const float* dhp; const float* mask; bf16_t* do2; const bf16_t* d3T; const bf16_t* dpre; bf16_t* dtd; const bf16_t* d0T;
+  const bf16_t* dP; long long lddp; const bf16_t* w1abT; const float* DOin;
+  const float* xhat; const float* rstd; float* DO;
+  bf16_t* DO16; const bf16_t* n3T; const bf16_t* upre; bf16_t* du; const bf16_t* n0T; bf16_t* dmi;
+};
+int launch_gnn_chain_bwd(const GnnChainBwd& a, int head, int tail, hipStream_t s);
 
 int launch_silu_fwd(const float* x, float* y, long long n, hipStream_t s);
 int launch_silu_bwd(const float* x, const float* dy, float* dx, long long n, int accumulate, hipStream_t s);
```

After: 50370 molecules/s (median of 6 runs). No clear change (+0.4%).
